# Sukikui/PTI-LDM-VAE

Hardware: AMD Instinct MI355X
Metric: vae_train_images_per_sec_256x256 (higher is better)
Workload: dtype fp16 forward operands + activations / bf16 backward operands + gradients, fp32 accumulate; 1 GPU; config/vae_dente_no_adv.json 256x256x1 batch 32/GPU: fwd + L1 + 1e-3*KL + bwd + all-reduce + Adam (perceptual term omitted: --perceptual times it; adversarial branch inactive before epoch 6, --adv times it); global_batch=32, parallelism=dp1

## Files before the change

### include/pti_vae.h

```cpp
#ifndef PTI_VAE_H
#define PTI_VAE_H

#include <stdint.h>

#ifdef __cplusplus
extern "C" {
#endif

typedef void* pti_stream_t;

#define PTI_ABI_VERSION 5

#define PTI_OK 0
#define PTI_EINVAL (-1)
#define PTI_EUNSUPPORTED (-2)
#define PTI_ELAUNCH (-3)

#define PTI_CONV_S1 0
#define PTI_CONV_S2PAD 1
#define PTI_CONV_UP2 2
#define PTI_CONV_ZINS 3

#define PTI_PRO_NONE 0
#define PTI_PRO_GN 1
#define PTI_PRO_GN_SILU 2

typedef struct pti_conv_desc {
  int32_t n, h, w, cin;
  int32_t ho, wo, cout;
  int32_t ksize;
  int32_t mode;
  int32_t prologue;
  int32_t groups;
  int32_t add_residual;
  int32_t accum_stats;
  int32_t out_groups;
  float eps;
  int32_t in_f32;
  int32_t out_f32;
  int64_t in_stride[4];
  int64_t out_stride[4];
  int32_t in_f16, res_f16, out_f16;
  int32_t pool2x2_out;
  int32_t w_f16;
  int32_t relu_out;
} pti_conv_desc;

int pti_abi_version(void);
const char* pti_last_error_string(void);
const char* pti_last_kernel_name(void);

int64_t pti_conv_packed_bytes(int cout, int cin, int ksize, int mode);
int pti_conv_pack_weights(const float* const* w_oihw, int nsrc, void* packed, int cout, int cin,
                          int ksize, int mode, int transpose_flip, int w_f16, pti_stream_t s);

int pti_conv_pack_entry_bytes(void);
int pti_conv_pack_table_fill(void* host_entry, const float* w_oihw_dev, void* packed_dev, int cout,
                             int cin, int ksize, int mode, int transpose_flip, int w_f16, int64_t* nblocks);
int pti_conv_pack_weights_batched(const void* table_dev, const int* blk_first_dev, int n,
                                  int total_blocks, pti_stream_t s);

int pti_gn_stats(const void* x_nhwc_16bit, int64_t* stats, int n, int hw, int c, int groups,
                 int x_f16, pti_stream_t s);

int pti_conv2d_mfma(const void* x, const void* w_packed, const float* bias, const int64_t* in_stats,
                    const float* gamma, const float* beta, const void* residual, void* y,
                    int64_t* out_stats, const pti_conv_desc* d, pti_stream_t s);

int pti_conv2d_mfma_saveact(const void* x, const void* w_packed, const float* bias, const int64_t* in_stats,
                            const float* gamma, const float* beta, const void* residual, void* y,
                            int64_t* out_stats, void* act_out, const pti_conv_desc* d, pti_stream_t s);

int pti_conv2d_direct(const void* x, const float* w_tck, const float* bias, const int64_t* in_stats,
                      const float* gamma, const float* beta, void* y, const pti_conv_desc* d,
                      pti_stream_t s);

#define PTI_DIRECT_REPACK_MAX 8
typedef struct {
  const float* w; const float* b;
  float* w_tck; float* w_tck_t; float* wpad; float* bpad;
  int cout, cin, pad_cin, reserved;
} pti_direct_repack_entry;
typedef struct {
  pti_direct_repack_entry e[PTI_DIRECT_REPACK_MAX];
  int n;
} pti_direct_repack_table;
int pti_direct_repack(const pti_direct_repack_table* t, pti_stream_t s);

int pti_wgrad_direct(const void* wide, const void* narrow, float* dw, float* dbias_wide,
                     float* dbias_narrow, const int64_t* in_stats, const float* gamma,
                     const float* beta, int n, int h, int w, int cw, int cn, int ksize, int sgn,
                     int prologue, int groups, float eps, int narrow_f32, int wide_f16,
                     const int64_t* narrow_stride, int64_t dw_stride_tap, int64_t dw_stride_cw,
                     int64_t dw_stride_k, void* workspace, int64_t workspace_bytes, pti_stream_t s);

int64_t pti_conv_wgrad_workspace_bytes(int cout, int cin, int ksize, int splits);
int pti_conv_wgrad_mfma(const void* x, const void* dy, const int64_t* in_stats, const float* gamma,
                        const float* beta, float* dw, float* dbias, void* workspace,
                        int64_t workspace_bytes, int accumulate, const pti_conv_desc* d,
                        pti_stream_t s);
int pti_conv_wgrad_mfma_partials(const void* x, const void* dy, const int64_t* in_stats,
                                 const float* gamma, const float* beta, void* workspace,
                                 int64_t workspace_bytes, const pti_conv_desc* d, int* splits_out,
                                 pti_stream_t s);
int pti_conv_wgrad_reduce(const void* workspace, int splits, float* dw, float* dbias,
                          int accumulate, const pti_conv_desc* d, pti_stream_t s);

#define PTI_WGRAD_BATCH_MAX 16
typedef struct pti_wgrad_job {
  const void* x;
  const void* dy;
  float* dw;
  float* dbias;
  int32_t n, h, w, cin, cout;
  int32_t accumulate;
} pti_wgrad_job;
int pti_conv_wgrad_mfma_batched(const pti_wgrad_job* jobs, int njobs, void* workspace, int64_t workspace_bytes,
                                pti_stream_t s);
int pti_conv_wgrad_batched_mode(int n, int h, int w, int cin, int cout);

int pti_gn_bwd_blocks(int n, int hw, int c);
int pti_gn_bwd(const void* x, const void* da, const void* dres, void* dx, const int64_t* stats,
               const float* gamma, const float* beta, float* sums, float* partials, float* dgamma,
               float* dbeta, int n, int hw, int c, int groups, float eps, int silu, int x_f16,
               pti_stream_t s);
int pti_conv_gnbwd_tiles(const pti_conv_desc* d);
int pti_conv_gnbwd_chain_supported(int cin, int cout, int ksize);
int pti_conv2d_mfma_gnbwd_chain(const void* g_in, const void* x_in, int x_in_f16, const int64_t* in_stats,
                                const float* in_gamma, const float* in_sums, void* dx_in_out, const void* w_packed,
                                const void* gx, const int64_t* gstats, const float* ggamma, const float* gbeta,
                                void* dy_out, float* gsums, const pti_conv_desc* d, int silu, pti_stream_t s);
int pti_gn_affine_grads(const float* sums, float* dgamma, float* dbeta, int n, int c, pti_stream_t s);
int pti_gn_sums_finalize_affine(const float* partials, float* sums, int n, int tiles, int row_len, const float* affine_sums,
                                float* dgamma, float* dbeta, int affine_c, pti_stream_t s);
int pti_conv2d_mfma_gnbwd(const void* dy_in, const void* w_packed, const void* gx, const int64_t* gstats,
                          const float* ggamma, const float* gbeta, void* dy_out, float* gpartials,
                          const pti_conv_desc* d, int silu, pti_stream_t s);
int pti_gn_sums_finalize(const float* partials, float* sums, int n, int tiles, int row_len,
                         pti_stream_t s);
int pti_gn_bwd_apply(const void* x, const void* dy, const void* dres, void* dx, const int64_t* stats,
                     const float* gamma, const float* beta, const float* sums, float* dgamma,
                     float* dbeta, int n, int hw, int c, int groups, float eps, int x_f16,
                     pti_stream_t s);
int pti_pool2x2_sum(const void* x, void* y, int n, int h, int w, int c, pti_stream_t s);

int pti_attention_fwd(const void* qkv, void* o, float* lse2, int b, int l, int c, pti_stream_t s);
int pti_attention_bwd(const void* qkv, const void* o, const void* dout, const float* lse2,
                      float* delta, void* dqkv, int b, int l, int c, pti_stream_t s);

int pti_latent_head_fwd(const float* h, const float* eps, const float* wm, const float* bm,
                        const float* wl, const float* bl, const float* wp, const float* bp,
                        float* mu, float* sigma, float* logvar, float* zq, int b, int hw, int l,
                        pti_stream_t s);
int pti_post_quant(const float* z_nchw, const float* wp, const float* bp, float* zq_nhwc, int b,
                   int hw, int l, pti_stream_t s);
#define PTI_POST_QUANT_BWD_MAX_BLOCKS 256
#define PTI_POST_QUANT_BWD_WS_FLOATS(l) (PTI_POST_QUANT_BWD_MAX_BLOCKS * ((l) * (l) + (l)))
int pti_post_quant_bwd(const float* dzq_nhwc, const float* z_nchw, const float* wp, float* dz_nchw,
                       float* gwp, float* gbp, float* workspace, int b, int hw, int l,
                       pti_stream_t s);
#define PTI_LATENT_BWD_MAX_BLOCKS 512
#define PTI_LATENT_BWD_WS_FLOATS(l) (PTI_LATENT_BWD_MAX_BLOCKS * 3 * ((l) * (l) + (l)))
int pti_latent_head_bwd(const float* h, const float* eps, const float* wm, const float* bm,
                        const float* wl, const float* bl, const float* wp, const float* bp,
                        const float* dzq, const float* dmu, const float* dsigma, float* dh,
                        float* gwm, float* gbm, float* gwl, float* gbl, float* gwp, float* gbp,
                        float* workspace, int b, int hw, int l, pti_stream_t s);

#define PTI_VAE_LOSS_MAX_BLOCKS 1024
#define PTI_VAE_LOSS_WS_FLOATS (2 * PTI_VAE_LOSS_MAX_BLOCKS)
int pti_vae_loss(const float* recon, const float* images, int64_t npix, const float* mu,
                 const float* third, int64_t nlat, int batch, float* out2, float* d_recon,
                 float* d_mu, float* d_third, float* workspace, int l2, int third_mode,
                 float kl_weight, pti_stream_t s);
// ... 184 lines not shown
```

### pti_ldm_vae_amd/_lib.py

```python
from __future__ import annotations

import ctypes as C
import os

_HERE = os.path.dirname(os.path.abspath(__file__))
LIB_PATH = os.environ.get("PTI_VAE_LIB") or os.path.join(_HERE, "libpti_vae_hip.so")

def env_overrides() -> dict:
    return {k: v for k, v in sorted(os.environ.items()) if k.startswith("PTI_")}


def refuse_wrong_result_env(who: str) -> None:
    bad = [k for k in os.environ if k.startswith("PTI_") and ("DIAG" in k or k == "PTI_ALLOW_WRONG_RESULTS")]
    if bad:
        raise SystemExit(f"{who}: refusing to run with wrong-result diagnostic variable(s) set: {sorted(bad)} "
                         "(timing diagnostics live in tools/diag_skip.py)")


ABI_VERSION = 5
PTI_CONV_S1, PTI_CONV_S2PAD, PTI_CONV_UP2, PTI_CONV_ZINS = 0, 1, 2, 3
PTI_PRO_NONE, PTI_PRO_GN, PTI_PRO_GN_SILU = 0, 1, 2


class ConvDesc(C.Structure):

    _fields_ = [
        ("n", C.c_int32), ("h", C.c_int32), ("w", C.c_int32), ("cin", C.c_int32),
        ("ho", C.c_int32), ("wo", C.c_int32), ("cout", C.c_int32),
        ("ksize", C.c_int32), ("mode", C.c_int32), ("prologue", C.c_int32), ("groups", C.c_int32),
        ("add_residual", C.c_int32), ("accum_stats", C.c_int32), ("out_groups", C.c_int32),
        ("eps", C.c_float), ("in_f32", C.c_int32), ("out_f32", C.c_int32),
        ("in_stride", C.c_int64 * 4), ("out_stride", C.c_int64 * 4),
        ("in_f16", C.c_int32), ("res_f16", C.c_int32), ("out_f16", C.c_int32), ("pool2x2_out", C.c_int32),
        ("w_f16", C.c_int32), ("relu_out", C.c_int32),
    ]


class WgradJob(C.Structure):

    _fields_ = [("x", C.c_void_p), ("dy", C.c_void_p), ("dw", C.c_void_p), ("dbias", C.c_void_p),
                ("n", C.c_int32), ("h", C.c_int32), ("w", C.c_int32), ("cin", C.c_int32), ("cout", C.c_int32),
                ("accumulate", C.c_int32)]


WGRAD_BATCH_MAX = 16
DIRECT_REPACK_MAX = 8
MASK_COMPARE_COLUMNS = ("n_gt", "n_pred", "components_gt", "components_pred", "kept_gt", "kept_pred", "filled_pred",
                        "intersection", "union", "gt_x", "gt_y", "gt_w", "gt_h", "pred_x", "pred_y", "pred_w", "pred_h",
                        "gt_width_upper", "gt_width_middle", "gt_width_lower",
                        "pred_width_upper", "pred_width_middle", "pred_width_lower", "status")
MASK_MOMENTS_COLUMNS = ("m00", "m10", "m01", "m20", "m11", "m02", "A", "B", "C", "status")
ALIGN_BOTTOM_COLUMNS = ("centre_gt", "centre_pred", "count_gt", "count_pred", "shift", "status")
GRAD_GUARD_COLUMNS = ("applied_steps", "skipped_steps", "sumsq", "norm", "coef", "skip", "bias1", "bias2_sqrt",
                      "ema_decay", "grad_mul")
GRAD_GUARD_HOST_COLUMNS = 8
GRAD_GUARD_PARTIALS_CAP = 1024


class DirectRepackEntry(C.Structure):

    _fields_ = [("w", C.c_void_p), ("b", C.c_void_p), ("w_tck", C.c_void_p), ("w_tck_t", C.c_void_p), ("wpad", C.c_void_p),
                ("bpad", C.c_void_p), ("cout", C.c_int32), ("cin", C.c_int32), ("pad_cin", C.c_int32), ("reserved", C.c_int32)]


class DirectRepackTable(C.Structure):

    _fields_ = [("e", DirectRepackEntry * DIRECT_REPACK_MAX), ("n", C.c_int32)]


_P = C.c_void_p
_I = C.c_int
_I64 = C.c_int64
_F = C.c_float
_D = C.c_double
_U32 = C.c_uint32

SIGNATURES = {
    "pti_abi_version": (_I, []),
    "pti_last_error_string": (C.c_char_p, []),
    "pti_last_kernel_name": (C.c_char_p, []),
    "pti_conv_packed_bytes": (_I64, [_I, _I, _I, _I]),
    "pti_conv_pack_weights": (_I, [C.POINTER(_P), _I, _P, _I, _I, _I, _I, _I, _I, _P]),
    "pti_conv_pack_entry_bytes": (_I, []),
    "pti_conv_pack_table_fill": (_I, [_P, _P, _P, _I, _I, _I, _I, _I, _I, C.POINTER(_I64)]),
    "pti_conv_pack_weights_batched": (_I, [_P, _P, _I, _I, _P]),
    "pti_gn_stats": (_I, [_P, _P, _I, _I, _I, _I, _I, _P]),
    "pti_conv2d_mfma": (_I, [_P, _P, _P, _P, _P, _P, _P, _P, _P, C.POINTER(ConvDesc), _P]),
    "pti_conv2d_mfma_saveact": (_I, [_P, _P, _P, _P, _P, _P, _P, _P, _P, _P, C.POINTER(ConvDesc), _P]),
    "pti_conv2d_direct": (_I, [_P, _P, _P, _P, _P, _P, _P, C.POINTER(ConvDesc), _P]),
    "pti_wgrad_direct": (_I, [_P, _P, _P, _P, _P, _P, _P, _P, _I, _I, _I, _I, _I, _I, _I, _I, _I, _F, _I, _I,
                              C.POINTER(_I64), _I64, _I64, _I64, _P, _I64, _P]),
    "pti_conv_wgrad_workspace_bytes": (_I64, [_I, _I, _I, _I]),
    "pti_conv_wgrad_mfma": (_I, [_P, _P, _P, _P, _P, _P, _P, _P, _I64, _I, C.POINTER(ConvDesc), _P]),
    "pti_conv_wgrad_mfma_partials": (_I, [_P, _P, _P, _P, _P, _P, _I64, C.POINTER(ConvDesc), C.POINTER(_I), _P]),
    "pti_conv_wgrad_mfma_batched": (_I, [C.POINTER(WgradJob), _I, _P, _I64, _P]),
    "pti_conv_wgrad_batched_mode": (_I, [_I, _I, _I, _I, _I]),
    "pti_direct_repack": (_I, [C.POINTER(DirectRepackTable), _P]),
    "pti_conv_wgrad_reduce": (_I, [_P, _I, _P, _P, _I, C.POINTER(ConvDesc), _P]),
    "pti_gn_bwd_blocks": (_I, [_I, _I, _I]),
    "pti_gn_bwd": (_I, [_P, _P, _P, _P, _P, _P, _P, _P, _P, _P, _P, _I, _I, _I, _I, _F, _I, _I, _P]),
    "pti_conv_gnbwd_tiles": (_I, [C.POINTER(ConvDesc)]),
    "pti_gn_sums_finalize": (_I, [_P, _P, _I, _I, _I, _P]),
    "pti_conv2d_mfma_gnbwd": (_I, [_P, _P, _P, _P, _P, _P, _P, _P, C.POINTER(ConvDesc), _I, _P]),
    "pti_conv_gnbwd_chain_supported": (_I, [_I, _I, _I]),
    "pti_conv2d_mfma_gnbwd_chain": (_I, [_P, _P, _I, _P, _P, _P, _P, _P, _P, _P, _P, _P, _P, _P, C.POINTER(ConvDesc), _I, _P]),
    "pti_gn_affine_grads": (_I, [_P, _P, _P, _I, _I, _P]),
    "pti_gn_sums_finalize_affine": (_I, [_P, _P, _I, _I, _I, _P, _P, _P, _I, _P]),
    "pti_gn_bwd_apply": (_I, [_P, _P, _P, _P, _P, _P, _P, _P, _P, _P, _I, _I, _I, _I, _F, _I, _P]),
    "pti_pool2x2_sum": (_I, [_P, _P, _I, _I, _I, _I, _P]),
    "pti_attention_fwd": (_I, [_P, _P, _P, _I, _I, _I, _P]),
    "pti_attention_bwd": (_I, [_P, _P, _P, _P, _P, _P, _I, _I, _I, _P]),
    "pti_latent_head_fwd": (_I, [_P] * 12 + [_I, _I, _I, _P]),
    "pti_post_quant": (_I, [_P, _P, _P, _P, _I, _I, _I, _P]),
    "pti_post_quant_bwd": (_I, [_P, _P, _P, _P, _P, _P, _P, _I, _I, _I, _P]),
    "pti_latent_head_bwd": (_I, [_P] * 19 + [_I, _I, _I, _P]),
    "pti_vae_loss": (_I, [_P, _P, _I64, _P, _P, _I64, _I, _P, _P, _P, _P, _P, _I, _I, _F, _P]),
    "pti_ar_vae_loss": (_I, [_P, _I, _I, _I, _P, _P, _P, _I, _P, _F, _P, _P, _P, _P]),
    "pti_pd_im2col_image": (_I, [_P, _P, _I, _I, _I, _P]),
    "pti_pd_im2col": (_I, [_P, _P, _P, _I, _I, _I, _I, _I, _I, _F, _P]),
    "pti_pd_in_stats": (_I, [_P, _P, _I, _I, _I, _F, _P]),
    "pti_pd_col2im_blocks": (_I, [_I, _I, _I]),
    "pti_pd_col2im": (_I, [_P, _P, _P, _P, _P, _I, _I, _I, _I, _I, _F, _P]),
    "pti_pd_col2im_image": (_I, [_P, _P, _I, _I, _I, _F, _I, _P]),
    "pti_pd_in_bwd_apply": (_I, [_P, _P, _P, _P, _P, _I, _I, _I, _P]),
    "pti_pd_lsgan_blocks": (_I, [_I]),
    "pti_pd_lsgan": (_I, [_P, _I, _I, _I, _F, _F, _F, _P, _P, _P]),
    "pti_pd_final_fwd": (_I, [_P, _P, _P, _P, _P, _I, _I, _I, _I, _F, _P]),
    "pti_pd_final_dgrad": (_I, [_P, _P, _P, _P, _P, _P, _I, _I, _I, _I, _F, _P]),
    "pti_pd_final_wgrad_blocks": (_I, [_I, _I, _I]),
    "pti_pd_final_wgrad": (_I, [_P, _P, _P, _P, _I, _I, _I, _I, _F, _P]),
    "pti_lpips_tap_blocks": (_I, [_I, _I]),
    "pti_lpips_tap_fwd": (_I, [_P, _P, _P, _P, _P, _I, _I, _I, _P]),
    "pti_lpips_tap_bwd": (_I, [_P, _P, _P, _P, _P, _P, _I, _I, _I, _P]),
    "pti_relu_f16": (_I, [_P, _I64, _P]),
    "pti_relu_bwd": (_I, [_P, _P, _I64, _P]),
    "pti_relu_bwd_add": (_I, [_P, _P, _P, _I64, _P]),
    "pti_maxpool3s2_out": (_I, [_I]),
    "pti_maxpool3s2_fwd": (_I, [_P, _P, _I, _I, _I, _I, _P]),
    "pti_maxpool3s2_bwd": (_I, [_P, _P, _P, _P, _I, _I, _I, _I, _I, _P]),
    "pti_squeeze_conv1_fwd": (_I, [_P, _P, _P, _I, _I, _I, _P]),
    "pti_squeeze_conv1_bwd": (_I, [_P, _P, _P, _P, _I, _I, _I, _P]),
    "pti_nchw_f32_to_nhwc_f16": (_I, [_P, _P, _I, _I, _I, _P]),
    "pti_pad_nchw_to_nhwc32": (_I, [_P, _P, _P, _I, _I, _I, _I, _I, _P]),
    "pti_slice_nhwc32_to_nchw": (_I, [_P, _P, _I, _I, _I, _I, _P]),
    "pti_nhwc_bf16_add_to_nchw_f32": (_I, [_P, _P, _I, _I, _I, _P]),
    "pti_lpips_tap_nhwc_blocks": (_I, [_I, _I]),
    "pti_lpips_tap_nhwc_fwd": (_I, [_P, _P, _P, _P, _P, _I, _I, _I, _P]),
    "pti_lpips_tap_nhwc_bwd": (_I, [_P, _P, _P, _P, _P, _P, _I, _I, _I, _P]),
    "pti_adam_step": (_I, [_P, _P, _P, _P, _I64, _F, _F, _F, _F, _I, _F, _P]),
    "pti_grad_guard_partials": (_I, [_I64]),
    "pti_grad_guard": (_I, [_P, _I64, _D, _D, _I, _F, _F, _D, _P, _P, _P]),
    "pti_adam_step_guarded": (_I, [_P, _P, _P, _P, _P, _I64, _F, _F, _F, _F, _P, _P]),
    "pti_preprocess_batch": (_I, [_P, _P, _P, _I, _I, _I, _P, _P, _P]),
    "pti_cast_nchw_f32_to_nhwc_bf16": (_I, [_P, _P, _I, _I, _I, _P]),
    "pti_cast_nhwc_bf16_to_nchw_f32": (_I, [_P, _P, _I, _I, _I, _P]),
    "pti_image_metrics_ws_floats": (_I64, [_I, _I, _I, _I]),
    "pti_image_metrics": (_I, [_P, _P, _I, _I, _I, _I, _I, _F, _F, _F, _F, _F, _P, _P, _P, _P]),
    "pti_latent_pairwise_ws_floats": (_I64, [_I, _I, _I]),
    "pti_latent_pairwise": (_I, [_P, _I64, _I, _P, _I64, _I, _I, _P, _I, _P, _I64, _P, _P]),
    "pti_latent_group_stats_ws_floats": (_I64, [_I, _I, _I, _I]),
    "pti_latent_group_stats": (_I, [_P, _I64, _I, _P, _P, _I64, _I, _P, _I, _I, _P, _P, _P]),
    "pti_mask_geometry": (_I, [_P, _P, _P, _I, _I, _I, _P, _I, _P, _I, _P, _P, _P, _P]),
    "pti_mlp_head_ws_floats": (_I64, [_I, _I, C.POINTER(C.c_int32), _I]),
    "pti_mlp_head_fwd": (_I, [_P, _I64, _I, _I, _P, C.POINTER(C.c_int32), _I, _I, _P, _P, _P, _I, _P, _P, _P, _P]),
    "pti_regression_metrics": (_I, [_P, _P, _P, _I, _I, _I, _P, _P]),
    "pti_elastic_field": (_I, [_P, _P, _F, _I, _I, _I, _P, _P]),
    "pti_augment_warp": (_I, [_P, _P, _P, _I, _I, _I, _I, _P, _P]),
    "pti_tsne_affinities_ws_floats": (_I64, [_I]),
    "pti_tsne_affinities": (_I, [_P, _I64, _I, _F, _P, _I64, _P, _P, _P]),
    "pti_tsne_step_ws_floats": (_I64, [_I, _I]),
    "pti_tsne_step": (_I, [_P, _I64, _I, _I, _P, _P, _P, _P, _P, _F, _F, _F, _P, _I, _P, _P]),
    "pti_umap_knn": (_I, [_P, _I64, _I, _I, _P, _P, _P]),
    "pti_umap_graph_capacity": (_I64, [_I, _I]),
# ... 65 lines not shown
```

### pti_ldm_vae_amd/csrc/conv_mfma.hip

```cpp
#include "conv_common.h"

namespace {
using namespace pti_conv;

constexpr int TH = 8, TW = 16;

__host__ __device__ constexpr int pick_cout_tile(int cout) { return cout % 128 == 0 ? 128 : (cout % 64 == 0 ? 64 : 32); }
__host__ __device__ constexpr int pick_ck(int cin, int stride2) {
  int ck = cin % 128 == 0 ? 128 : (cin % 64 == 0 ? 64 : 32);
  return (stride2 && ck > 64) ? 64 : ck;
}
__host__ __device__ constexpr int pick_wblk(int kbc, int nt) {
  int best = 1;
  for (int w = 1; w <= kbc; ++w)
    if (kbc % w == 0 && w * nt <= 16) best = w;
  return best;
}

template <int KS, int S, int CK, int COUT_TILE>
struct Cfg {
  static constexpr int HH = (TH - 1) * S + KS, HW = (TW - 1) * S + KS;
  static constexpr int NP = HH * HW;
  static constexpr int NC = CK / 8;
  static constexpr int PIXB = CK * 2;
// ... 112 lines not shown
      const int vy = vy0 + hy, vx = vx0 + hx;
      bool v = (p < C::NP) && vy >= 0 && vy < VH && vx >= 0 && vx < VW;
      int iy = vy, ix = vx;
      if (twox) {
        if (a.mode == PTI_CONV_ZINS) v = v && !((vy | vx) & 1);
        iy = vy >> 1;
        ix = vx >> 1;
      }
      ok[it] = v;
      raw[it] = u32x4{0u, 0u, 0u, 0u};
      if (v) raw[it] = *(const u32x4*)(a.x + ((size_t)(n * a.H + iy) * a.W + ix) * a.Cin + chunk * CK + lc * 8);
    }
#pragma unroll
    for (int it = 0; it < C::HITERS; ++it) {
      const int p = lp0 + it * PSTEP;
      if (p < C::NP) {
        const int hy = p / C::HW, hx = p - hy * C::HW;
        u32x4 r = raw[it];
        if (a.prologue != PTI_PRO_NONE && ok[it]) {
          float f[8];
          unpack8f(r, f, a.in_f16);
#pragma unroll
          for (int j = 0; j < 8; ++j) {
            float v = f[j] * sc[j] + sh[j];
            if (a.prologue == PTI_PRO_GN_SILU) v = silu_f(v);
            f[j] = v;
          }
          r = OPH ? pack8f(f, true) : pack8(f);
        } else if (a.in_f16 && !OPH) {
          float f[8];
          unpack8f(r, f, true);
          r = pack8(f);
        }
        const int key = (hx >> C::KEY_SHIFT) & (C::NC - 1);
        *(u32x4*)(halo + p * C::PIXB + ((lc ^ key) << 4)) = r;
      }
    }
    __syncthreads();

#pragma unroll
    for (int s = 0; s < C::NSTEP; ++s) {
      const int g = chunk * C::NSTEP + s;
      const bool more = (g + 1 < total_steps);
      if (more) wload(g + 1);
      const unsigned char* wcur = wbuf + (g & 1) * C::STEPB;
#pragma unroll
      for (int kbl = 0; kbl < C::WBLK; ++kbl) {
        constexpr int dummy = 0;
        (void)dummy;
        const int kb = s * C::WBLK + kbl;
        const int tap = kb / C::KPC, kc = kb % C::KPC;
        const int kh = tap / KS, kw = tap % KS;
        bf16x8 bfrag[C::PXF], afrag[C::CF];
#pragma unroll
        for (int i = 0; i < C::PXF; ++i)
          bfrag[i] = *(const bf16x8*)(halo + pbase[i][kw] + kh * C::HW * C::PIXB + ((kc * 32) ^ tkey[kw]));
#pragma unroll
        for (int c = 0; c < C::CF; ++c)
          afrag[c] = *(const bf16x8*)(wcur + ((kbl * C::NT + wn * C::CF + c) * 64 + lane) * 16);
#pragma unroll
        for (int i = 0; i < C::PXF; ++i)
#pragma unroll
          for (int c = 0; c < C::CF; ++c)
            acc[i][c] = mfma32<OPH>(afrag[c], bfrag[i], acc[i][c]);
      }
      if (more) wstore((g + 1) & 1);
      __syncthreads();
    }
  }

  const int j = lane & 31;
  stat_t* sstat = reinterpret_cast<stat_t*>(smem);
  const bool do_stats = a.out_stats != nullptr;
  const int ocpg = do_stats ? a.Cout / a.out_groups : 1;
  if (do_stats) {
    if (tid < 2 * a.out_groups) sstat[tid] = 0;
    __syncthreads();
  }
#pragma unroll
  for (int i = 0; i < C::PXF; ++i) {
    const int ty = 2 * (wm * C::PXF + i) + (j >> 4), tx = j & 15;
    const int oy = oy0 + ty, ox = ox0 + tx;
    const bool inb = (oy < a.Ho) && (ox < a.Wo);
    const size_t pix = ((size_t)(n * a.Ho + oy) * a.Wo + ox) * a.Cout;
#pragma unroll
    for (int c = 0; c < C::CF; ++c) {
#pragma unroll
      for (int q = 0; q < 4; ++q) {
        const int co = ct * COUT_TILE + (wn * C::CF + c) * 32 + 8 * q + 4 * hsel;
        float v0 = acc[i][c][4 * q + 0], v1 = acc[i][c][4 * q + 1], v2 = acc[i][c][4 * q + 2],
              v3 = acc[i][c][4 * q + 3];
        if (a.bias) {
          const f32x4 b = *(const f32x4*)(a.bias + co);
          v0 += b[0]; v1 += b[1]; v2 += b[2]; v3 += b[3];
        }
        u32x2 packed = u32x2{0u, 0u};
        if (inb) {
          if (a.res) {
            const u32x2 rr = *(const u32x2*)(a.res + pix + co);
            float e0, e1, e2, e3;
            unpack2f(rr[0], a.res_f16, e0, e1);
            unpack2f(rr[1], a.res_f16, e2, e3);
            v0 += e0; v1 += e1; v2 += e2; v3 += e3;
          }
          packed = pack4f(v0, v1, v2, v3, a.out_f16);
          *(u32x2*)(a.y + pix + co) = packed;
        }
        if (do_stats) {
          float r0, r1, r2, r3;
          unpack2f(packed[0], a.out_f16, r0, r1);
          unpack2f(packed[1], a.out_f16, r2, r3);
          if (!inb) r0 = r1 = r2 = r3 = 0.f;
          if (ocpg >= 4) {
            float s1 = (r0 + r1) + (r2 + r3), s2 = (r0 * r0 + r1 * r1) + (r2 * r2 + r3 * r3);
#pragma unroll
            for (int o = 16; o > 0; o >>= 1) {
              s1 += __shfl_xor(s1, o, 64);
              s2 += __shfl_xor(s2, o, 64);
            }
            if (j == 0) {
              const int g = co / ocpg;
              stat_add(&sstat[2 * g], s1);
              stat_add(&sstat[2 * g + 1], s2);
            }
          } else {
            float a1 = r0 + r1, a2 = r0 * r0 + r1 * r1, b1 = r2 + r3, b2 = r2 * r2 + r3 * r3;
#pragma unroll
            for (int o = 16; o > 0; o >>= 1) {
              a1 += __shfl_xor(a1, o, 64);
              a2 += __shfl_xor(a2, o, 64);
              b1 += __shfl_xor(b1, o, 64);
              b2 += __shfl_xor(b2, o, 64);
            }
            if (j == 0) {
              const int g = co / 2;
              stat_add(&sstat[2 * g], a1);
              stat_add(&sstat[2 * g + 1], a2);
              stat_add(&sstat[2 * g + 2], b1);
              stat_add(&sstat[2 * g + 3], b2);
            }
          }
        }
      }
    }
  }
  if (do_stats) {
    __syncthreads();
    const int g0 = (ct * COUT_TILE) / ocpg, ng = COUT_TILE / ocpg;
    if (tid < 2 * ng)
      atomicAdd((unsigned long long*)&a.out_stats[(n * a.out_groups + g0) * 2 + tid], (unsigned long long)sstat[2 * g0 + tid]);
  }
}

template <int KS, int CK, int CT, int PXF, bool SAVE, int FM, int PRO>
__global__ __launch_bounds__(256, (PXF == 2 ? 4 : 2)) void conv_mfma2_kernel(ConvArgs a) {
  using C = Cfg2<KS, CK, CT, PXF>;
  const int prologue = PRO >= 0 ? PRO : a.prologue;
  const bool gn_on = FM == 3 ? true : (FM == 0 ? a.gn_mode != 0 : false);
  const bool in_f16 = FM == 0 ? (bool)a.in_f16 : (FM == 1);
  const bool res_f16 = FM == 0 ? (bool)a.res_f16 : (FM == 1 || FM == 3);
  const bool out_f16 = FM == 0 ? (bool)a.out_f16 : (FM == 1);
  constexpr bool OPH = (FM == 1);
  if (out_f16) fp16_saturate_on();
  __shared__ __attribute__((aligned(16))) unsigned char smem[C::LDS_BYTES];
  unsigned char* halo = smem;
  const int tid = threadIdx.x, lane = tid & 63, wave = tid >> 6;
  const int hsel = lane >> 5;
  int t = blockIdx.x;
  const int tile_x = t % a.tiles_x;
  t /= a.tiles_x;
  const int tile_y = t % a.tiles_y;
  const int n = t / a.tiles_y;
  const int oy0 = tile_y * C::TH2, ox0 = tile_x * C::TW2;
  const int ct = blockIdx.y;
  const int nchunks = a.Cin / CK;
  const int wm = wave / C::WN, wn = wave % C::WN;

  const int pad_lo = (a.mode == PTI_CONV_ZINS) ? 2 : (KS - 1) / 2;
  const int vy0 = oy0 - pad_lo, vx0 = ox0 - pad_lo;
  const bool twox = (a.mode == PTI_CONV_UP2) || (a.mode == PTI_CONV_ZINS);
  const int VH = twox ? 2 * a.H : a.H, VW = twox ? 2 * a.W : a.W;

  int pbase[KS], tkey[KS];
  {
    const int j = lane & 31, tx = j & 15, row0 = 2 * PXF * wm + (j >> 4);
#pragma unroll
    for (int kw = 0; kw < KS; ++kw) {
      const int hx = tx + kw;
      tkey[kw] = (hsel ^ ((hx >> C::KEY_SHIFT) & (C::NC - 1))) << 4;
      pbase[kw] = (row0 * C::HW + hx) * C::PIXB;
    }
  }
  f32x16 acc[PXF];
#pragma unroll
  for (int i = 0; i < PXF; ++i)
#pragma unroll
    for (int r = 0; r < 16; ++r) acc[i][r] = 0.f;

  const int lc = tid % C::NC, lp0 = tid / C::NC;
  constexpr int PSTEP = 256 / C::NC;
  const int cpg = a.Cin / (a.groups > 0 ? a.groups : 1);
  reinterpret_cast<float*>(smem + C::STAT_OFF)[tid] = 0.f;
  float* sfl = reinterpret_cast<float*>(smem + C::STAT_OFF + 1024);
  if (prologue == PTI_PRO_GN || prologue == PTI_PRO_GN_SILU) {
    if (tid < 2 * a.groups) sfl[tid] = stat_f(a.in_stats, n * a.groups * 2 + tid);
  } else if (gn_on) {
    if (tid < 2 * a.g_groups) sfl[tid] = stat_f(a.g_stats, n * a.g_groups * 2 + tid);
  }
  float gq = 0.f, bq = 0.f;
  if (gn_on) {
    if (tid < CT) {
      gq = a.g_gamma[ct * CT + tid];
      bq = a.g_beta[ct * CT + tid];
    }
  } else if (a.bias) {
    if (tid < CT) reinterpret_cast<float*>(smem + C::BIAS_OFF)[tid] = a.bias[ct * CT + tid];
  }
  if (a.res) {
#pragma unroll
    for (int it = 0; it < C::EITERS; ++it) {
      const int slot = it * 256 + tid;
      const int p = slot / C::ENC, c = slot % C::ENC;
      const int oy = oy0 + p / C::TW2, ox = ox0 + p % C::TW2;
      if (oy < a.Ho && ox < a.Wo) {
        const bf16* src = a.res + ((size_t)(n * a.Ho + oy) * a.Wo + ox) * a.Cout + ct * CT + ((c ^ ((p >> 2) & (C::ENC - 1))) << 3);
        __builtin_amdgcn_global_load_lds((const __attribute__((address_space(1))) void*)src,
                                         (__attribute__((address_space(3))) void*)(smem + C::RT_OFF + (it * 256 + wave * 64) * 16),
                                         16, 0, 0);
      }
    }
  }

  const int epc = tid % C::ENC, epp0 = tid / C::ENC;
  constexpr int EPSTEP = 256 / C::ENC;

  for (int chunk = 0; chunk < nchunks; ++chunk) {
    const unsigned char* wlane =
        a.w + ((size_t)(ct * nchunks + chunk) * C::KBC * C::NT + wn) * 1024 + lane * 16;
    bf16x8 wa[C::R], wb[C::R];
    auto wload = [&](bf16x8 (&dst)[C::R], int g) {
#pragma unroll
      for (int u = 0; u < C::R; ++u) {
        int kb = g * C::R + u;
        kb = kb < C::KBC ? kb : C::KBC - 1;
        dst[u] = *(const bf16x8*)(wlane + (size_t)kb * C::NT * 1024);
      }
    };
    constexpr bool WLATE = (SAVE && PXF == 2) || PRO == PRO_GNB;
    if constexpr (!WLATE) wload(wa, 0);

    u32x4 raw[C::HITERS];
    u32x4 raw2[PRO == PRO_GNB ? C::HITERS : 1];
    bool ok[C::HITERS];
    {
      const __amdgpu_buffer_rsrc_t xrs = __builtin_amdgcn_make_buffer_rsrc(
          const_cast<bf16*>(a.x), 0, (unsigned)a.N * (unsigned)a.H * (unsigned)a.W * (unsigned)a.Cin * 2u, 0x00020000);
      const __amdgpu_buffer_rsrc_t x2rs = __builtin_amdgcn_make_buffer_rsrc(
          const_cast<bf16*>(PRO == PRO_GNB ? a.x2 : a.x), 0, (unsigned)a.N * (unsigned)a.H * (unsigned)a.W * (unsigned)a.Cin * 2u, 0x00020000);
      const unsigned base = ((unsigned)n * a.H * a.W * a.Cin + chunk * CK + lc * 8) * 2u;
      const unsigned rowb = (unsigned)a.W * a.Cin * 2u, pixb = (unsigned)a.Cin * 2u;
#pragma unroll
      for (int it = 0; it < C::HITERS; ++it) {
        const int p = lp0 + it * PSTEP;
        const int hy = p / C::HW, hx = p - hy * C::HW;
        const int vy = vy0 + hy, vx = vx0 + hx;
        bool v = (p < C::NP) && (unsigned)vy < (unsigned)VH && (unsigned)vx < (unsigned)VW;
        int iy = vy, ix = vx;
        if (twox) {
          if (a.mode == PTI_CONV_ZINS) v = v && !((vy | vx) & 1);
          iy = vy >> 1;
          ix = vx >> 1;
        }
        ok[it] = v;
        const unsigned off = v ? base + (unsigned)iy * rowb + (unsigned)ix * pixb : 0x80000000u;
        raw[it] = __builtin_bit_cast(u32x4, __builtin_amdgcn_raw_buffer_load_b128(xrs, off, 0, 0));
        if constexpr (PRO == PRO_GNB) raw2[it] = __builtin_bit_cast(u32x4, __builtin_amdgcn_raw_buffer_load_b128(x2rs, off, 0, 0));
      }
    }
    if (chunk == 0) __syncthreads();
    float sc[8], sh[8];
    [[maybe_unused]] float gnb_b = 0.f, gnb_d = 0.f;
    if constexpr (PRO == PRO_GNB) {
      const int ch0 = chunk * CK + lc * 8, g = ch0 / cpg;
      const float mean = stat_f(a.in_stats, (n * a.groups + g) * 2) * a.inv_cnt;
      const float rstd = rsqrtf(fmaxf(stat_f(a.in_stats, (n * a.groups + g) * 2 + 1) * a.inv_cnt - mean * mean, 0.f) + a.eps);
      float t1 = 0.f, t2 = 0.f;
      for (int cc = g * cpg; cc < (g + 1) * cpg; ++cc) {
        const f32x2 sv = *(const f32x2*)(a.p_sums + ((size_t)n * a.Cin + cc) * 2);
        const float gm = a.gamma[cc];
        t1 += gm * sv[0];
        t2 += gm * sv[1];
      }
      const float c1 = t1 * a.inv_cnt, c2 = t2 * a.inv_cnt;
#pragma unroll
      for (int j = 0; j < 8; ++j) sc[j] = rstd * a.gamma[ch0 + j];
      gnb_b = -rstd * rstd * c2;
      gnb_d = -rstd * c1 - gnb_b * mean;
    } else if (prologue != PTI_PRO_NONE) {
      float mu_[8], rs_[8];
      gn_params<8>(sfl, a.gamma, a.beta, chunk * CK + lc * 8, cpg, a.inv_cnt, a.eps, sc, sh, mu_, rs_);
    }
    if (chunk > 0) __syncthreads();
#pragma unroll
    for (int it = 0; it < C::HITERS; ++it) {
      const int p = lp0 + it * PSTEP;
      if (p < C::NP) {
        const int hy = p / C::HW, hx = p - hy * C::HW;
        u32x4 r = raw[it];
        if constexpr (PRO == PRO_GNB) {
          if (ok[it]) {
            float f[8], h[8];
            unpack8(r, f);
            unpack8f(raw2[it], h, a.x2_f16 != 0);
#pragma unroll
            for (int j = 0; j < 8; ++j) f[j] = fmaf(sc[j], f[j], fmaf(gnb_b, h[j], gnb_d));
            r = pack8(f);
          }
        } else if (prologue != PTI_PRO_NONE && ok[it]) {
          float f[8];
          unpack8f(r, f, in_f16);
          if (PXF == 4 && prologue == PTI_PRO_GN_SILU) {
#pragma unroll
            for (int j = 0; j < 8; j += 2) {
              const f32x2 o = gn_silu2(f32x2{f[j], f[j + 1]}, f32x2{sc[j], sc[j + 1]}, f32x2{sh[j], sh[j + 1]});
              f[j] = o[0];
              f[j + 1] = o[1];
            }
          } else {
#pragma unroll
            for (int j = 0; j < 8; ++j) {
              float v = f[j] * sc[j] + sh[j];
              if (prologue == PTI_PRO_GN_SILU) v = silu_f(v);
              f[j] = v;
            }
          }
          r = OPH ? pack8f(f, true) : pack8(f);
        } else if (in_f16 && !OPH) {
          float f[8];
          unpack8f(r, f, true);
          r = pack8(f);
        }
        const int key = (hx >> C::KEY_SHIFT) & (C::NC - 1);
        *(u32x4*)(halo + p * C::PIXB + ((lc ^ key) << 4)) = r;
      }
    }
    __syncthreads();

    if constexpr (SAVE) {
      if (ct == 0) {
        constexpr int PL = (KS - 1) / 2;
        constexpr int SITERS = C::TH2 * C::TW2 * C::NC / 256;
        const __amdgpu_buffer_rsrc_t srs = __builtin_amdgcn_make_buffer_rsrc(
            a.act_out, 0, (unsigned)a.N * (unsigned)a.H * (unsigned)a.W * (unsigned)a.Cin * 2u, 0x00020000);
#pragma unroll 1
        for (int it = 0; it < SITERS; ++it) {
          const int idx = tid + it * 256;
          const int c8 = idx % C::NC, pi = idx / C::NC;
          const int hy = pi / C::TW2 + PL, hx = pi % C::TW2 + PL;
          const int vy = vy0 + hy, vx = vx0 + hx;
          if (vy < a.H && vx < a.W) {
            const int key = (hx >> C::KEY_SHIFT) & (C::NC - 1);
            u32x4 piece = *(const u32x4*)(halo + (hy * C::HW + hx) * C::PIXB + ((c8 ^ key) << 4));
            if constexpr (OPH) {
              float f[8];
              unpack8f(piece, f, true);
              piece = pack8(f);
            }
            __builtin_amdgcn_raw_buffer_store_b128(__builtin_bit_cast(bu32x4, piece), srs,
                                                   ((unsigned)((n * a.H + vy) * a.W + vx) * a.Cin + chunk * CK + c8 * 8) * 2u, 0, 2 );
          }
        }
      }
    }

    if constexpr (WLATE) wload(wa, 0);
    const int txl = lane & 15;
    auto baddr = [&](int kb) -> const unsigned char* {
      kb = kb < C::KBC ? kb : C::KBC - 1;
      const int tap = kb / C::KPC, kc = kb - tap * C::KPC;
      const int kh = (KS == 3) ? tap / 3 : 0, kw = tap - kh * KS;
      const int hx = txl + kw;
      const int tk = (hsel ^ ((hx >> C::KEY_SHIFT) & (C::NC - 1))) << 4;
      return halo + pbase[0] + (kh * C::HW + kw) * C::PIXB + ((kc * 32) ^ tk);
    };
    bf16x8 b0[PXF], b1[PXF];
    auto bread = [&](bf16x8 (&dst)[PXF], int kb) {
      const unsigned char* bp = baddr(kb);
#pragma unroll
      for (int i = 0; i < PXF; ++i) dst[i] = *(const bf16x8*)(bp + 2 * i * C::HW * C::PIXB);
    };
    auto group = [&](const bf16x8 (&w)[C::R], int g) {
      const int kb0 = g * C::R;
#pragma unroll
      for (int u = 0; u < C::R; ++u) {
        if ((u & 1) == 0) {
          bread(b1, kb0 + u + 1);
#pragma unroll
          for (int i = 0; i < PXF; ++i) acc[i] = mfma32<OPH>(w[u], b0[i], acc[i]);
        } else {
          bread(b0, kb0 + u + 1);
#pragma unroll
          for (int i = 0; i < PXF; ++i) acc[i] = mfma32<OPH>(w[u], b1[i], acc[i]);
        }
      }
      if (C::R & 1) {
#pragma unroll
        for (int i = 0; i < PXF; ++i) b0[i] = b1[i];
      }
    };
    constexpr int NG = C::KBC / C::R;
    bread(b0, 0);
    if constexpr (NG == 1) {
      group(wa, 0);
    } else {
#pragma clang loop unroll(disable)
      for (int g = 0; g < NG; g += 2) {
        wload(wb, g + 1);
        group(wa, g);
        wload(wa, g + 2);
        group(wb, g + 1);
      }
    }
  }

  const int j = lane & 31;
  unsigned char* etile = smem;
  const bool do_stats = (FM == 2 || FM == 3) ? false : a.out_stats != nullptr;
  const int ocpg = do_stats ? a.Cout / a.out_groups : 1;
  __syncthreads();
  float* gtab = reinterpret_cast<float*>(smem + C::GT_OFF);
  if (gn_on) {
    if (tid < CT) {
      gtab[tid] = gq;
      gtab[CT + tid] = bq;
    }
    __syncthreads();
  }
  const unsigned char* rtile = smem + C::RT_OFF;
  const int col0 = wn * 32 + 4 * hsel;
  float st1[4] = {0.f, 0.f, 0.f, 0.f}, st2[4] = {0.f, 0.f, 0.f, 0.f};
  float su1[4] = {0.f, 0.f, 0.f, 0.f}, su2[4] = {0.f, 0.f, 0.f, 0.f};
  if (gn_on) {
    const int gcpg = a.Cout / a.g_groups;
    float* gsm = reinterpret_cast<float*>(smem + C::STAT_OFF);
    float L[32];
#pragma unroll
    for (int q = 0; q < 4; ++q) {
      const int col = col0 + 8 * q, ch0 = ct * CT + col;
      float scv[4], shv[4], muv[4], rsv[4], l1[4] = {0.f, 0.f, 0.f, 0.f}, l2[4] = {0.f, 0.f, 0.f, 0.f};
      gn_params<4>(sfl, gtab - ct * CT, gtab + CT - ct * CT, ch0, gcpg, a.g_inv_cnt, a.g_eps, scv, shv, muv, rsv);
      float nmr[4];
#pragma unroll
      for (int r = 0; r < 4; ++r) nmr[r] = -muv[r] * rsv[r];
#pragma unroll
      for (int i = 0; i < PXF; ++i) {
        const int p = (2 * PXF * wm + 2 * i + (j >> 4)) * 16 + (j & 15);
        const bool inb = (oy0 + (p >> 4) < a.Ho) && (ox0 + (p & 15) < a.Wo);
        unsigned char* ep = etile + p * C::EPITCH + col * 2;
        const u32x2 rr = *(const u32x2*)(rtile + p * (CT * 2) + ((((col >> 3) ^ (p >> 2)) & (C::ENC - 1)) << 4) + (col & 7) * 2);
        float xv[4];
        unpack2f(rr[0], res_f16, xv[0], xv[1]);
        unpack2f(rr[1], res_f16, xv[2], xv[3]);
        float dv[4];
#pragma unroll
        for (int r = 0; r < 4; ++r) {
          float v = acc[i][4 * q + r];
          if (a.gn_mode == 2) v *= dsilu_f(xv[r] * scv[r] + shv[r]);
          dv[r] = v;
        }
        const u32x2 packed = pack4(dv[0], dv[1], dv[2], dv[3]);
        *(u32x2*)ep = packed;
        if (inb) {
#pragma unroll
          for (int r = 0; r < 4; ++r) {
            l1[r] += dv[r];
            l2[r] = fmaf(dv[r], fmaf(xv[r], rsv[r], nmr[r]), l2[r]);
          }
        }
      }
#pragma unroll
      for (int r = 0; r < 4; ++r) {
        L[8 * q + 2 * r] = l1[r];
        L[8 * q + 2 * r + 1] = l2[r];
      }
    }
    fold32<32>(L, j);
    gsm[wm * 2 * CT + col0 * 2 + 16 * (j >> 3) + (j & 7)] = L[0];
  } else {
#pragma unroll
  for (int i = 0; i < PXF; ++i) {
    const int p = (2 * PXF * wm + 2 * i + (j >> 4)) * 16 + (j & 15);
    const bool inb = (oy0 + (p >> 4) < a.Ho) && (ox0 + (p & 15) < a.Wo);
#pragma unroll
    for (int q = 0; q < 4; ++q) {
      const int col = col0 + 8 * q;
      float v0 = acc[i][4 * q + 0], v1 = acc[i][4 * q + 1], v2 = acc[i][4 * q + 2], v3 = acc[i][4 * q + 3];
      if (a.bias) {
        const f32x4 b = *(const f32x4*)(smem + C::BIAS_OFF + col * 4);
        v0 += b[0]; v1 += b[1]; v2 += b[2]; v3 += b[3];
      }
      unsigned char* ep = etile + p * C::EPITCH + col * 2;
      if (a.res) {
        const u32x2 rr = *(const u32x2*)(rtile + p * (CT * 2) + ((((col >> 3) ^ (p >> 2)) & (C::ENC - 1)) << 4) + (col & 7) * 2);
        float e0, e1, e2, e3;
        unpack2f(rr[0], res_f16, e0, e1);
        unpack2f(rr[1], res_f16, e2, e3);
        v0 += e0; v1 += e1; v2 += e2; v3 += e3;
      }
      if constexpr (FM == 1 && PRO == PTI_PRO_NONE) {
        if (a.relu_out) { v0 = fmaxf(v0, 0.f); v1 = fmaxf(v1, 0.f); v2 = fmaxf(v2, 0.f); v3 = fmaxf(v3, 0.f); }
      }
      const u32x2 packed = pack4f(v0, v1, v2, v3, out_f16);
      *(u32x2*)ep = packed;
      if (do_stats && inb) {
        float r0, r1, r2, r3;
        unpack2f(packed[0], out_f16, r0, r1);
        unpack2f(packed[1], out_f16, r2, r3);
        if (ocpg >= 4) {
          st1[q] += (r0 + r1) + (r2 + r3);
          st2[q] += (r0 * r0 + r1 * r1) + (r2 * r2 + r3 * r3);
        } else {
          st1[q] += r0 + r1; st2[q] += r0 * r0 + r1 * r1;
          su1[q] += r2 + r3; su2[q] += r2 * r2 + r3 * r3;
        }
      }
    }
  }
  }
  if (do_stats) {
    stat_t* sstat = reinterpret_cast<stat_t*>(smem + C::STAT_OFF);
    if (ocpg >= 4) {
      float v[8];
#pragma unroll
      for (int q = 0; q < 4; ++q) { v[2 * q] = st1[q]; v[2 * q + 1] = st2[q]; }
      fold32<8>(v, j);
      if ((j & 3) == 0) {
        const int idx = j >> 2, q = idx >> 1;
        const int g = (ct * CT + col0 + 8 * q) / ocpg;
        stat_add(&sstat[2 * g + (idx & 1)], v[0]);
      }
    } else {
      float v[16];
#pragma unroll
      for (int q = 0; q < 4; ++q) { v[4 * q] = st1[q]; v[4 * q + 1] = st2[q]; v[4 * q + 2] = su1[q]; v[4 * q + 3] = su2[q]; }
      fold32<16>(v, j);
      if ((j & 1) == 0) {
        const int idx = j >> 1, q = idx >> 2;
        const int g = (ct * CT + col0 + 8 * q) / 2;
        stat_add(&sstat[2 * g + (idx & 3)], v[0]);
      }
    }
  }
  __syncthreads();
  const __amdgpu_buffer_rsrc_t yrs = __builtin_amdgcn_make_buffer_rsrc(
      a.y, 0, ((unsigned)a.N * (unsigned)a.Ho * (unsigned)a.Wo * (unsigned)a.Cout * 2u) >> (a.pool2 ? 2 : 0), 0x00020000);
  if ((FM == 0 || FM == 2) && a.pool2) {
    constexpr int PITERS = (C::EITERS + 3) / 4;
#pragma unroll
    for (int it = 0; it < PITERS; ++it) {
      const int idx = tid + it * 256;
      const int c8 = idx % C::ENC, pp = idx / C::ENC;
      const int py = pp / 8, px = pp % 8;
      const int oy = (oy0 >> 1) + py, ox = (ox0 >> 1) + px;
      if (pp < C::MPX / 4 && oy < (a.Ho >> 1) && ox < (a.Wo >> 1)) {
        const unsigned char* src = etile + ((2 * py) * 16 + 2 * px) * C::EPITCH + c8 * 16;
        float s_[8], f_[8];
        unpack8f(*(const u32x4*)src, s_, out_f16);
        unpack8f(*(const u32x4*)(src + C::EPITCH), f_, out_f16);
#pragma unroll
        for (int q = 0; q < 8; ++q) s_[q] += f_[q];
        unpack8f(*(const u32x4*)(src + 16 * C::EPITCH), f_, out_f16);
#pragma unroll
        for (int q = 0; q < 8; ++q) s_[q] += f_[q];
        unpack8f(*(const u32x4*)(src + 17 * C::EPITCH), f_, out_f16);
#pragma unroll
        for (int q = 0; q < 8; ++q) s_[q] += f_[q];
        __builtin_amdgcn_raw_buffer_store_b128(__builtin_bit_cast(bu32x4, pack8f(s_, out_f16)), yrs,
                                               ((unsigned)((n * (a.Ho >> 1) + oy) * (a.Wo >> 1) + ox) * a.Cout + ct * CT + c8 * 8) * 2u, 0, 2);
      }
    }
  } else
#pragma unroll
  for (int it = 0; it < C::EITERS; ++it) {
    const int p = epp0 + it * EPSTEP;
    const int oy = oy0 + (p >> 4), ox = ox0 + (p & 15);
    if (oy < a.Ho && ox < a.Wo)
      __builtin_amdgcn_raw_buffer_store_b128(__builtin_bit_cast(bu32x4, *(const u32x4*)(etile + p * C::EPITCH + epc * 16)), yrs,
                                             ((unsigned)((n * a.Ho + oy) * a.Wo + ox) * a.Cout + ct * CT + epc * 8) * 2u, 0, 2);
  }
  if (gn_on) {
    if (tid < 2 * CT) {
      const float* gsm = reinterpret_cast<const float*>(smem + C::STAT_OFF);
      float v = gsm[tid];
#pragma unroll
      for (int m = 1; m < C::WM; ++m) v += gsm[m * 2 * CT + tid];
      a.g_sums[(((size_t)n * a.g_T + tile_y * a.tiles_x + tile_x) * a.Cout + ct * CT) * 2 + tid] = v;
    }
  } else if (do_stats) {
    const stat_t* sstat = reinterpret_cast<const stat_t*>(smem + C::STAT_OFF);
    const int g0 = (ct * CT) / ocpg, ng = CT / ocpg;
    if (tid < 2 * ng)
      atomicAdd((unsigned long long*)&a.out_stats[(n * a.out_groups + g0) * 2 + tid], (unsigned long long)sstat[2 * g0 + tid]);
  }
}

template <int KS, int CK, int CT, int PXF>
int launch2_cfg(ConvArgs a, hipStream_t st) {
  using C = Cfg2<KS, CK, CT, PXF>;
  a.tiles_x = cdiv(a.Wo, C::TW2);
  a.tiles_y = cdiv(a.Ho, C::TH2);
  a.g_T = a.tiles_x * a.tiles_y;
  dim3 grid(a.N * a.tiles_x * a.tiles_y, a.Cout / CT);
  const bool res = a.res != nullptr;
  const int fm = (a.w_f16 && a.in_f16 && a.out_f16 && (a.res_f16 || !res)) ? 1
               : (!a.in_f16 && !a.out_f16 && (!a.res_f16 || !res)) ? 2
               : (!a.in_f16 && !a.out_f16 && a.res_f16) ? 3 : 0;
  const bool fwd_silu = fm == 1 && a.prologue == PTI_PRO_GN_SILU && !a.gn_mode && !a.pool2;
  const bool fwd_plain = fm == 1 && a.prologue == PTI_PRO_NONE && !a.gn_mode && !a.pool2;
  const bool dgrad = fm == 2 && a.prologue == PTI_PRO_NONE && !a.gn_mode && !a.out_stats;
  const bool dgrad_gn = fm == 3 && a.prologue == PTI_PRO_NONE && a.gn_mode && !a.out_stats && !a.pool2;
  if (a.x2) {
    if constexpr (KS == 3 && PXF == 4 && CT == 128) {
      if (!(fm == 3 && a.gn_mode && a.act_out && !a.out_stats && !a.pool2 && a.mode == PTI_CONV_S1 && !a.relu_out)) return 4;
      PTI_LAUNCH((conv_mfma2_kernel<KS, CK, CT, PXF, true, 3, PRO_GNB>), grid, dim3(256), 0, st, a);
      return 0;
    } else {
      return 4;
    }
  }
  if (a.relu_out && !(fwd_plain && !a.act_out)) return 3;
  constexpr int FPRO = PXF == 4 ? PTI_PRO_GN_SILU : -1;
  const bool fwd_gn_rt = fm == 1 && a.prologue == PTI_PRO_GN && !a.gn_mode && !a.pool2 && FPRO < 0;
  if constexpr (KS == 3) {
    if (a.act_out) {
      if (fwd_silu || fwd_gn_rt) PTI_LAUNCH((conv_mfma2_kernel<KS, CK, CT, PXF, true, 1, FPRO>), grid, dim3(256), 0, st, a);
      else if (a.w_f16) return 2;
      else PTI_LAUNCH((conv_mfma2_kernel<KS, CK, CT, PXF, true, 0, -1>), grid, dim3(256), 0, st, a);
      return 0;
    }
  } else if (a.act_out) {
    return 1;
  }
  if (fwd_silu) PTI_LAUNCH((conv_mfma2_kernel<KS, CK, CT, PXF, false, 1, FPRO>), grid, dim3(256), 0, st, a);
  else if (fwd_plain) PTI_LAUNCH((conv_mfma2_kernel<KS, CK, CT, PXF, false, 1, PTI_PRO_NONE>), grid, dim3(256), 0, st, a);
  else if (fm == 1 && !a.gn_mode && !a.pool2) PTI_LAUNCH((conv_mfma2_kernel<KS, CK, CT, PXF, false, 1, -1>), grid, dim3(256), 0, st, a);
  else if (a.w_f16) return 2;
  else if (dgrad) PTI_LAUNCH((conv_mfma2_kernel<KS, CK, CT, PXF, false, 2, PTI_PRO_NONE>), grid, dim3(256), 0, st, a);
  else if (dgrad_gn) PTI_LAUNCH((conv_mfma2_kernel<KS, CK, CT, PXF, false, 3, PTI_PRO_NONE>), grid, dim3(256), 0, st, a);
  else PTI_LAUNCH((conv_mfma2_kernel<KS, CK, CT, PXF, false, 0, -1>), grid, dim3(256), 0, st, a);
  return 0;
}
template <int KS>
int launch2(const ConvArgs& a, int ck, int ct, hipStream_t st) {
  if (ct == 128) {
    if (ck == 128) return launch2_cfg<KS, 128, 128, 4>(a, st);
    if (ck == 64) return launch2_cfg<KS, 64, 128, 4>(a, st);
    return launch2_cfg<KS, 32, 128, 4>(a, st);
  }
  if (ct == 64) {
    if (ck == 64) return launch2_cfg<KS, 64, 64, 2>(a, st);
    return launch2_cfg<KS, 32, 64, 2>(a, st);
  }
  return launch2_cfg<KS, 32, 32, 2>(a, st);
}

struct PackArgs {
  const float* src[4];
  int nsrc;
  bf16* dst;
  int cout_l, cin_l;
  int cout_o, cin_o;
  int ks, ck, cout_tile, flip;
  int f16;
  long long total;
};

__device__ __forceinline__ void pack_eight(const PackArgs& p, int e8) {
  const int NT = p.cout_tile / 32, KPC = p.ck / 16, KBC = p.ks * p.ks * KPC, nch = p.cin_l / p.ck;
  int r = e8;
  const int lane = r % 64; r /= 64;
  const int nt = r % NT; r /= NT;
  const int kb = r % KBC; r /= KBC;
  const int chunk = r % nch;
  const int ct = r / nch;
  const int co = ct * p.cout_tile + nt * 32 + (lane & 31);
  const int tap = kb / KPC, kc = kb % KPC;
  const int ci0 = chunk * p.ck + kc * 16 + 8 * (lane >> 5);
  const int kk = p.ks * p.ks;
  const float* src;
  size_t stride;
  if (!p.flip) {
    const int s_ = co / p.cout_o, cs = co % p.cout_o;
    src = p.src[s_] + ((size_t)cs * p.cin_o + ci0) * kk + tap;
    stride = kk;
  } else {
    src = p.src[0] + ((size_t)ci0 * p.cin_o + co) * kk + (kk - 1 - tap);
    stride = (size_t)p.cin_o * kk;
  }
  float f[8];
#pragma unroll
  for (int j = 0; j < 8; ++j) f[j] = src[j * stride];
  *(u32x4*)(p.dst + (size_t)e8 * 8) = p.f16 ? pack8f(f, true) : pack8(f);
}

__global__ void pack_weights_kernel(PackArgs p) {
  if (p.f16) fp16_saturate_on();
  const long long e8 = (long long)blockIdx.x * blockDim.x + threadIdx.x;
  if (e8 * 8 < p.total) pack_eight(p, (int)e8);
}

__global__ void pack_weights_batched_kernel(const PackArgs* __restrict__ table, const int* __restrict__ blk_first, int n) {
  int lo = 0, hi = n - 1;
  const int b = blockIdx.x;
  while (lo < hi) {
    const int mid = (lo + hi + 1) >> 1;
    if (blk_first[mid] <= b) lo = mid; else hi = mid - 1;
  }
  const PackArgs p = table[lo];
  if (p.f16) fp16_saturate_on();
  const int e8 = (b - blk_first[lo]) * 256 + threadIdx.x;
  if ((long long)e8 * 8 < p.total) pack_eight(p, e8);
}

template <int KS, int S, int CK, int COUT_TILE>
int launch_cfg(const ConvArgs& a, hipStream_t st) {
  dim3 grid(a.N * a.tiles_x * a.tiles_y, a.Cout / COUT_TILE);
  if (a.w_f16) PTI_LAUNCH((conv_mfma_kernel<KS, S, CK, COUT_TILE, true>), grid, dim3(256), 0, st, a);
  else PTI_LAUNCH((conv_mfma_kernel<KS, S, CK, COUT_TILE, false>), grid, dim3(256), 0, st, a);
  return 0;
}

template <int KS, int S, int CK>
int launch_ct(const ConvArgs& a, int cout_tile, hipStream_t st) {
  switch (cout_tile) {
    case 128: return launch_cfg<KS, S, CK, 128>(a, st);
    case 64: return launch_cfg<KS, S, CK, 64>(a, st);
    default: return launch_cfg<KS, S, CK, 32>(a, st);
  }
}

template <int KS, int S>
int launch_ck(const ConvArgs& a, int ck, int cout_tile, hipStream_t st) {
  static_assert(S == 2, "the v1 kernel is kept for the stride-2 gather only");
  switch (ck) {
    case 64: return launch_ct<KS, S, 64>(a, cout_tile, st);
    default: return launch_ct<KS, S, 32>(a, cout_tile, st);
  }
}

}

extern "C" int64_t pti_conv_packed_bytes(int cout, int cin, int ksize, int mode) {
  (void)mode;
  if (cout <= 0 || cin <= 0 || cout % 32 || cin % 32 || (ksize != 1 && ksize != 3)) return 0;
  return (int64_t)2 * cout * cin * ksize * ksize;
}

extern "C" int pti_conv_pack_weights(const float* const* w, int nsrc, void* packed, int cout, int cin,
                                     int ksize, int mode, int transpose_flip, int w_f16, pti_stream_t s) {
  if (!w || !packed || nsrc < 1 || nsrc > 4) PTI_FAIL(PTI_EINVAL, "pack_weights: bad pointer/nsrc");
  if (cout % 32 || cin % 32 || (ksize != 1 && ksize != 3))
    PTI_FAIL(PTI_EUNSUPPORTED, "pack_weights: cout=%d cin=%d k=%d need multiples of 32, k in {1,3}", cout, cin, ksize);
  if (transpose_flip && nsrc != 1) PTI_FAIL(PTI_EINVAL, "pack_weights: transpose_flip needs nsrc=1");
  PackArgs p;
  for (int i = 0; i < 4; ++i) p.src[i] = i < nsrc ? w[i] : nullptr;
  p.nsrc = nsrc;
  p.dst = (bf16*)packed;
  p.cout_o = cout;
  p.cin_o = cin;
  p.cout_l = transpose_flip ? cin : cout * nsrc;
  p.cin_l = transpose_flip ? cout : cin;
  p.ks = ksize;
  p.flip = transpose_flip;
  p.f16 = w_f16 ? 1 : 0;
  p.cout_tile = pick_cout_tile(p.cout_l);
  p.ck = (mode == PTI_CONV_S2PAD) ? pick_ck(p.cin_l, true) : pick_ck2(p.cin_l, p.cout_tile);
  p.total = (long long)p.cout_l * p.cin_l * ksize * ksize;
  const int blocks = (int)((p.total + 2047) / 2048);
  PTI_LAUNCH(pack_weights_kernel, dim3(blocks), dim3(256), 0, (hipStream_t)s, p);
  PTI_CHECK_LAUNCH("pack_weights");
  return PTI_OK;
}

static int fill_pack(PackArgs& p, const float* w, void* packed, int cout, int cin, int ksize, int mode, int flip, int f16) {
  if (cout % 32 || cin % 32 || (ksize != 1 && ksize != 3)) return -1;
  for (int i = 0; i < 4; ++i) p.src[i] = nullptr;
  p.src[0] = w;
  p.nsrc = 1;
  p.dst = (bf16*)packed;
  p.cout_o = cout; p.cin_o = cin;
  p.cout_l = flip ? cin : cout;
  p.cin_l = flip ? cout : cin;
  p.ks = ksize; p.flip = flip; p.f16 = f16 ? 1 : 0;
  p.cout_tile = pick_cout_tile(p.cout_l);
  p.ck = (mode == PTI_CONV_S2PAD) ? pick_ck(p.cin_l, true) : pick_ck2(p.cin_l, p.cout_tile);
  p.total = (long long)p.cout_l * p.cin_l * ksize * ksize;
  return 0;
}

extern "C" int pti_conv_pack_entry_bytes(void) { return (int)sizeof(PackArgs); }
extern "C" int pti_conv_pack_table_fill(void* host_entry, const float* w, void* packed, int cout, int cin, int ksize,
                                        int mode, int transpose_flip, int w_f16, int64_t* nblocks) {
  if (!host_entry || !w || !packed || !nblocks) PTI_FAIL(PTI_EINVAL, "pack_table_fill: null pointer");
  PackArgs p;
  if (fill_pack(p, w, packed, cout, cin, ksize, mode, transpose_flip, w_f16))
    PTI_FAIL(PTI_EUNSUPPORTED, "pack_table_fill: cout=%d cin=%d k=%d", cout, cin, ksize);
  *(PackArgs*)host_entry = p;
  *nblocks = (p.total + 2047) / 2048;
  return PTI_OK;
}
extern "C" int pti_conv_pack_weights_batched(const void* table_dev, const int* blk_first_dev, int n, int total_blocks,
                                             pti_stream_t s) {
  if (!table_dev || !blk_first_dev || n <= 0 || total_blocks <= 0) PTI_FAIL(PTI_EINVAL, "pack_weights_batched: bad args");
  PTI_LAUNCH(pack_weights_batched_kernel, dim3(total_blocks), dim3(256), 0, (hipStream_t)s,
                     (const PackArgs*)table_dev, blk_first_dev, n);
  PTI_CHECK_LAUNCH("pack_weights_batched");
  return PTI_OK;
}

struct GnBwdFuse {
  int mode; const int64_t* stats; const float* gamma; const float* beta; float* sums;
  const void* x2 = nullptr; int x2_f16 = 0; const int64_t* p_stats = nullptr; const float* p_gamma = nullptr; const float* p_sums = nullptr;
};

static int conv2d_mfma_impl(const void* x, const void* w_packed, const float* bias, const int64_t* in_stats,
                            const float* gamma, const float* beta, const void* residual, void* y,
                            int64_t* out_stats, const pti_conv_desc* d, const GnBwdFuse* gf, void* act_out,
                            pti_stream_t s) {
  if (!x || !w_packed || !y || !d) PTI_FAIL(PTI_EINVAL, "conv2d_mfma: null pointer");
  const bool chain = gf && gf->x2;
  if (act_out && !chain && (d->mode != PTI_CONV_S1 || d->prologue == PTI_PRO_NONE || d->ksize != 3))
    PTI_FAIL(PTI_EUNSUPPORTED, "conv2d_mfma: the activated-input side output needs a 3x3 PTI_CONV_S1 launch with a GroupNorm prologue");
  if (d->cin % 32 || d->cout % 32 || d->cin <= 0 || d->cout <= 0)
    PTI_FAIL(PTI_EUNSUPPORTED, "conv2d_mfma: cin=%d cout=%d must be positive multiples of 32", d->cin, d->cout);
  if (d->ksize != 1 && d->ksize != 3) PTI_FAIL(PTI_EUNSUPPORTED, "conv2d_mfma: ksize %d", d->ksize);
  if (d->ksize == 1 && d->mode != PTI_CONV_S1) PTI_FAIL(PTI_EUNSUPPORTED, "conv2d_mfma: 1x1 supports PTI_CONV_S1 only");
  if (d->n <= 0 || d->h <= 0 || d->w <= 0) PTI_FAIL(PTI_EINVAL, "conv2d_mfma: bad dims");
  int eho, ewo;
  switch (d->mode) {
    case PTI_CONV_S1: eho = d->h; ewo = d->w; break;
    case PTI_CONV_S2PAD: eho = (d->h + 1 - 3) / 2 + 1; ewo = (d->w + 1 - 3) / 2 + 1; break;
    case PTI_CONV_UP2: case PTI_CONV_ZINS: eho = 2 * d->h; ewo = 2 * d->w; break;
    default: PTI_FAIL(PTI_EUNSUPPORTED, "conv2d_mfma: mode %d", d->mode);
  }
  if (d->ho != eho || d->wo != ewo)
    PTI_FAIL(PTI_EINVAL, "conv2d_mfma: output %dx%d does not match mode %d on %dx%d (want %dx%d)", d->ho, d->wo,
             d->mode, d->h, d->w, eho, ewo);
  if (d->prologue != PTI_PRO_NONE) {
    if (!in_stats || !gamma || !beta || d->groups <= 0 || d->cin % d->groups)
      PTI_FAIL(PTI_EINVAL, "conv2d_mfma: prologue needs stats/gamma/beta and groups | cin");
    if (d->groups > 32) PTI_FAIL(PTI_EUNSUPPORTED, "conv2d_mfma: prologue supports at most 32 groups");
  }
  if (d->add_residual && !residual) PTI_FAIL(PTI_EINVAL, "conv2d_mfma: add_residual without residual");
  if (d->accum_stats) {
    if (!out_stats || d->out_groups <= 0 || d->cout % d->out_groups) PTI_FAIL(PTI_EINVAL, "conv2d_mfma: bad out stats");
    const int ocpg = d->cout / d->out_groups;
    if (ocpg != 2 && (ocpg % 4 != 0 || ocpg > 32)) PTI_FAIL(PTI_EUNSUPPORTED, "conv2d_mfma: channels/group %d for fused stats", ocpg);
    if (d->out_groups > 64) PTI_FAIL(PTI_EUNSUPPORTED, "conv2d_mfma: fused statistics support at most 64 groups");
  }
  ConvArgs a;
  a.x = (const bf16*)x; a.w = (const unsigned char*)w_packed; a.bias = bias; a.in_stats = (const stat_t*)in_stats;
  a.gamma = gamma; a.beta = beta; a.res = d->add_residual ? (const bf16*)residual : nullptr; a.y = (bf16*)y;
  a.out_stats = d->accum_stats ? (stat_t*)out_stats : nullptr;
  a.N = d->n; a.H = d->h; a.W = d->w; a.Cin = d->cin; a.Ho = d->ho; a.Wo = d->wo; a.Cout = d->cout;
  a.mode = d->mode; a.prologue = d->prologue; a.groups = d->groups; a.out_groups = d->out_groups;
  a.gn_mode = 0; a.g_groups = 0; a.g_inv_cnt = 0.f; a.g_eps = 0.f;
  a.g_stats = nullptr; a.g_gamma = a.g_beta = nullptr; a.g_sums = nullptr; a.g_T = 0;
  a.act_out = (bf16*)act_out;
  a.in_f16 = d->in_f16; a.res_f16 = d->res_f16; a.out_f16 = d->out_f16;
  a.pool2 = d->pool2x2_out;
  a.w_f16 = d->w_f16;
  a.relu_out = d->relu_out;
  if (a.relu_out && (gf || d->mode == PTI_CONV_S2PAD))
    PTI_FAIL(PTI_EUNSUPPORTED, "conv2d_mfma: relu_out is for plain fp16 forward launches (stride-1 gather, no prologue)");
  if (a.w_f16 && !(d->in_f16 && d->out_f16 && (d->res_f16 || !d->add_residual)) )
    PTI_FAIL(PTI_EUNSUPPORTED, "conv2d_mfma: fp16-packed weights need fp16 input, output and residual (the forward convs)");
  if (a.w_f16 && (gf || d->pool2x2_out))
    PTI_FAIL(PTI_EUNSUPPORTED, "conv2d_mfma: fp16-packed weights are for forward launches only");
  if (a.pool2 && (d->mode == PTI_CONV_S2PAD || d->accum_stats || gf || (d->ho & 1) || (d->wo & 1)))
    PTI_FAIL(PTI_EUNSUPPORTED, "conv2d_mfma: pool2x2_out needs a stride-1 gather, even output size, no fused statistics");
  a.eps = d->eps;
  a.inv_cnt = d->prologue != PTI_PRO_NONE ? 1.0f / ((float)(d->cin / d->groups) * (float)d->h * (float)d->w) : 0.f;
  if (gf) {
    if (d->groups > 32) PTI_FAIL(PTI_EUNSUPPORTED, "conv2d_mfma_gnbwd: at most 32 groups");
    a.gn_mode = gf->mode; a.g_groups = d->groups; a.g_eps = d->eps;
    a.g_inv_cnt = 1.0f / ((float)(d->cout / d->groups) * (float)d->ho * (float)d->wo);
    a.g_stats = (const stat_t*)gf->stats; a.g_gamma = gf->gamma; a.g_beta = gf->beta; a.g_sums = gf->sums;
  }
  a.x2 = nullptr; a.p_sums = nullptr; a.x2_f16 = 0;
  if (chain) {
    if (!gf->p_stats || !gf->p_gamma || !gf->p_sums || !act_out || d->mode != PTI_CONV_S1 || d->ksize != 3 ||
        d->cin % d->groups || d->cin / d->groups < 8)
      PTI_FAIL(PTI_EINVAL, "conv2d_mfma_gnbwd_chain: bad arguments (3x3 stride-1, >= 8 channels per group)");
    a.x2 = (const bf16*)gf->x2; a.x2_f16 = gf->x2_f16; a.p_sums = gf->p_sums;
    a.in_stats = (const stat_t*)gf->p_stats; a.gamma = gf->p_gamma; a.groups = d->groups;
    a.inv_cnt = 1.0f / ((float)(d->cin / d->groups) * (float)d->h * (float)d->w);
  }
  if ((long long)d->n * d->ho * d->wo * d->cout * 2 >= (1ll << 31))
    PTI_FAIL(PTI_EUNSUPPORTED, "conv2d_mfma: output tensor of %lld bytes (the stores use 32-bit offsets: < 2 GiB)",
             (long long)d->n * d->ho * d->wo * d->cout * 2);
  if (d->mode != PTI_CONV_S2PAD && (long long)d->n * d->h * d->w * d->cin * 2 >= (1ll << 31))
    PTI_FAIL(PTI_EUNSUPPORTED, "conv2d_mfma: input tensor of %lld bytes (the halo loads use 32-bit offsets: < 2 GiB)",
             (long long)d->n * d->h * d->w * d->cin * 2);
  a.tiles_x = cdiv(d->wo, TW); a.tiles_y = cdiv(d->ho, TH);
  const int cout_tile = pick_cout_tile(d->cout);
  int rc, ck;
  if (d->mode == PTI_CONV_S2PAD) {
    ck = pick_ck(d->cin, true);
    rc = launch_ck<3, 2>(a, ck, cout_tile, (hipStream_t)s);
  } else {
    ck = pick_ck2(d->cin, cout_tile);
    rc = (d->ksize == 3 && d->cin == 128 && d->cout == 128 && !a.x2) ? launch_conv_ws128(a, (hipStream_t)s) : 1;
    if (rc == 1)
      rc = d->ksize == 1 ? launch2<1>(a, ck, cout_tile, (hipStream_t)s) : launch2<3>(a, ck, cout_tile, (hipStream_t)s);
  }
  if (rc == 3) PTI_FAIL(PTI_EUNSUPPORTED, "conv2d_mfma: relu_out needs a plain fp16 forward launch (w_f16, fp16 in/out, no prologue, no side output)");
  if (rc == 2) PTI_FAIL(PTI_EUNSUPPORTED, "conv2d_mfma: no fp16-operand kernel for this launch (w_f16 with this prologue / epilogue)");
  if (rc == 4) PTI_FAIL(PTI_EUNSUPPORTED, "conv2d_mfma_gnbwd_chain: only 3x3 launches on 128-wide input and output tiles with an fp16 GroupNorm input");
  if (rc != 0) PTI_FAIL(PTI_EUNSUPPORTED, "conv2d_mfma: no kernel for ck=%d cout_tile=%d", ck, cout_tile);
  PTI_CHECK_LAUNCH("conv2d_mfma");
  return PTI_OK;
}

extern "C" int pti_conv2d_mfma(const void* x, const void* w_packed, const float* bias, const int64_t* in_stats,
                               const float* gamma, const float* beta, const void* residual, void* y,
                               int64_t* out_stats, const pti_conv_desc* d, pti_stream_t s) {
  return conv2d_mfma_impl(x, w_packed, bias, in_stats, gamma, beta, residual, y, out_stats, d, nullptr, nullptr, s);
}

extern "C" int pti_conv2d_mfma_saveact(const void* x, const void* w_packed, const float* bias, const int64_t* in_stats,
                                       const float* gamma, const float* beta, const void* residual, void* y,
                                       int64_t* out_stats, void* act_out, const pti_conv_desc* d, pti_stream_t s) {
  if (!act_out) PTI_FAIL(PTI_EINVAL, "conv2d_mfma_saveact: null act_out");
  return conv2d_mfma_impl(x, w_packed, bias, in_stats, gamma, beta, residual, y, out_stats, d, nullptr, act_out, s);
}

extern "C" int pti_conv_gnbwd_tiles(const pti_conv_desc* d) {
  if (!d || d->cout % 32 || d->ho <= 0 || d->wo <= 0) return 0;
  const int ct = pick_cout_tile(d->cout);
  const int th = ct == 128 ? 8 : (ct == 64 ? 8 : 16);
  return cdiv(d->ho, th) * cdiv(d->wo, 16);
}

extern "C" int pti_conv_gnbwd_chain_supported(int cin, int cout, int ksize) {
  return ksize == 3 && cin % 128 == 0 && cout % 128 == 0;
}

extern "C" int pti_conv2d_mfma_gnbwd_chain(const void* g_in, const void* x_in, int x_in_f16, const int64_t* in_stats,
                                           const float* in_gamma, const float* in_sums, void* dx_in_out, const void* w_packed,
                                           const void* gx, const int64_t* gstats, const float* ggamma, const float* gbeta,
                                           void* dy_out, float* gsums, const pti_conv_desc* d, int silu, pti_stream_t s) {
  if (!g_in || !x_in || !in_stats || !in_gamma || !in_sums || !dx_in_out || !gx || !gstats || !ggamma || !gbeta || !gsums || !d)
    PTI_FAIL(PTI_EINVAL, "conv2d_mfma_gnbwd_chain: null pointer");
  if (d->mode != PTI_CONV_S1 || d->prologue != PTI_PRO_NONE || d->add_residual || d->accum_stats)
    PTI_FAIL(PTI_EUNSUPPORTED, "conv2d_mfma_gnbwd_chain: plain stride-1 data-gradient launches only");
  if (d->groups <= 0 || d->cout % d->groups || d->cin % d->groups) PTI_FAIL(PTI_EINVAL, "conv2d_mfma_gnbwd_chain: groups must divide cin and cout");
  GnBwdFuse gf{silu ? 2 : 1, gstats, ggamma, gbeta, gsums};
  gf.x2 = x_in; gf.x2_f16 = x_in_f16; gf.p_stats = in_stats; gf.p_gamma = in_gamma; gf.p_sums = in_sums;
  pti_conv_desc dd = *d;
  dd.add_residual = 1;
  return conv2d_mfma_impl(g_in, w_packed, nullptr, nullptr, nullptr, nullptr, gx, dy_out, nullptr, &dd, &gf, dx_in_out, s);
}

extern "C" int pti_conv2d_mfma_gnbwd(const void* dy_in, const void* w_packed, const void* gx, const int64_t* gstats,
                                     const float* ggamma, const float* gbeta, void* dy_out, float* gsums,
                                     const pti_conv_desc* d, int silu, pti_stream_t s) {
  if (!gx || !gstats || !ggamma || !gbeta || !gsums || !d) PTI_FAIL(PTI_EINVAL, "conv2d_mfma_gnbwd: null pointer");
  if (d->mode == PTI_CONV_S2PAD || d->prologue != PTI_PRO_NONE || d->add_residual || d->accum_stats)
    PTI_FAIL(PTI_EUNSUPPORTED, "conv2d_mfma_gnbwd: plain stride-1 / zero-insert data-gradient launches only");
  if (d->groups <= 0 || d->cout % d->groups) PTI_FAIL(PTI_EINVAL, "conv2d_mfma_gnbwd: groups must divide cout");
  GnBwdFuse gf{silu ? 2 : 1, gstats, ggamma, gbeta, gsums};
  pti_conv_desc dd = *d;
  dd.add_residual = 1;
  return conv2d_mfma_impl(dy_in, w_packed, nullptr, nullptr, nullptr, nullptr, gx, dy_out, nullptr, &dd, &gf, nullptr, s);
}
```

### pti_ldm_vae_amd/engine.py

```python
from __future__ import annotations

import contextlib
import gc
import os
import warnings

import torch

from . import ops
from .models import autoencoderkl as M
from .ops import (BF16, F32, PTI_CONV_S1, PTI_CONV_S2PAD, PTI_CONV_UP2, PTI_CONV_ZINS, PTI_PRO_GN, PTI_PRO_GN_SILU,
                  PTI_PRO_NONE)


class _Act:

    __slots__ = ("t", "stats")

    def __init__(self, t, stats=None):
        self.t, self.stats = t, stats


def _empty(shape, like, dtype=BF16):
    return torch.empty(shape, dtype=dtype, device=like.device)


@contextlib.contextmanager
def gc_off_for_capture():
    gc.collect()
    enabled = gc.isenabled()
    gc.disable()
    try:
        yield
    finally:
        if enabled:
            gc.enable()


def capture_or_eager(what, *bodies):
    graphs, results = [], []
    try:
        with gc_off_for_capture():
            for body in bodies:
                g = torch.cuda.CUDAGraph()
                with torch.cuda.graph(g, pool=graphs[0].pool() if graphs else None, capture_error_mode="thread_local"):
                    results.append(body(*results))
                graphs.append(g)
    except Exception as ex:
        warnings.warn(f"HIP-graph capture of {what} failed ({ex!r}); continuing with eager launches")
        torch.cuda.synchronize()
        return None
    return graphs, results


class _MfmaConv:

    def __init__(self, net, wname, bname, ksize, mode, fused_names=None, fwd_f16=True):
        self.net, self.ksize, self.mode = net, ksize, mode
        self.fwd_f16, self.f16 = fwd_f16, False
        self.wname, self.bname, self.fused = wname, bname, fused_names
        if fused_names:
            w0 = net._param_by_name[fused_names[0][0]]
            self.cout, self.cin = 3 * w0.shape[0], w0.shape[1]
        else:
            w = net._param_by_name[wname]
            self.cout, self.cin = w.shape[0], w.shape[1]
        self.wp = self.wpt = None

    def _w(self):
        if self.fused:
            o, n, _ = self.net._slots[self.fused[0][0]]
            return self.net._arena[o:o + 3 * n].view(self.cout, self.cin, 1, 1)
        return self.net._param_by_name[self.wname].data.view(self.cout, self.cin, self.ksize, self.ksize)

    def bias(self):
        if self.fused:
            o, n, _ = self.net._slots[self.fused[0][1]]
            return self.net._arena[o:o + 3 * n]
        return self.net._param_by_name[self.bname].data

    def grads(self):
        if self.fused:
            o, n, _ = self.net._slots[self.fused[0][0]]
            ob, nb, _ = self.net._slots[self.fused[0][1]]
            g = self.net.grad_arena
            return g[o:o + 3 * n], g[ob:ob + 3 * nb]
        return self.net.grad_view(self.wname).view(-1), self.net.grad_view(self.bname)

    def fwd(self, x, *, pro=PTI_PRO_NONE, norm=None, residual=None, want_stats=False, eng=None, act_out=None,
            out_dtype=None):
        n, h, w, _ = x.t.shape
        ho, wo = ops.conv_out_hw(h, w, self.mode)
        y = _empty((n, ho, wo, self.cout), x.t, out_dtype or eng.act_dtype)
        st = eng.new_stats(n) if want_stats else None
        g, b = (norm.weight.data, norm.bias.data) if norm is not None else (None, None)
        ops.conv_mfma(x.t, self.wp, self.bias(), y, cout=self.cout, ksize=self.ksize, mode=self.mode, prologue=pro,
                      in_stats=x.stats if pro else None, gamma=g, beta=b, groups=eng.G, eps=eng.eps,
                      residual=residual, out_stats=st, out_groups=eng.G, act_out=act_out)
        return _Act(y, st)

    def dgrad(self, dy, *, residual=None):
        n, ho, wo, _ = dy.shape
        if self.mode == PTI_CONV_S2PAD:
            out = _empty((n, 2 * ho, 2 * wo, self.cin), dy)
            ops.conv_mfma(dy, self.wpt, None, out, cout=self.cin, ksize=3, mode=PTI_CONV_ZINS, residual=residual)
            return out
        if self.mode == PTI_CONV_UP2:
            pooled = _empty((n, ho // 2, wo // 2, self.cin), dy)
            ops.conv_mfma(dy, self.wpt, None, pooled, cout=self.cin, ksize=self.ksize, mode=PTI_CONV_S1, pool2=True)
            return pooled
        out = _empty((n, ho, wo, self.cin), dy)
        ops.conv_mfma(dy, self.wpt, None, out, cout=self.cin, ksize=self.ksize, mode=PTI_CONV_S1, residual=residual)
        return out

    def dgrad_gn(self, dy, x, norm, *, silu, dres, eng):
        g, sums = self.dgrad_gn_raw(dy, x, norm, silu=silu, eng=eng)
        return self._gn_apply(g, sums, x, norm, dres, eng)

    def _gn_apply(self, g, sums, x, norm, dres, eng):
        dx = _empty(x.t.shape, x.t)
        ops.gn_bwd_apply(x.t, g, dx, x.stats, norm.weight.data, norm.bias.data, sums,
                         norm.net.grad_view(norm.prefix + ".weight"), norm.net.grad_view(norm.prefix + ".bias"),
                         groups=eng.G, eps=eng.eps, dres=dres)
        return dx

    def dgrad_gn_raw(self, dy, x, norm, *, silu, eng):
        n, ho, wo, _ = dy.shape
        g = _empty((n, ho, wo, self.cin), dy)
        sums = eng.zeros(n * self.cin * 2)
        ops.conv_mfma_gnbwd(dy, self.wpt, x.t, x.stats, norm.weight.data, norm.bias.data, g, sums, cout=self.cin,
                            ksize=self.ksize, mode=PTI_CONV_S1, groups=eng.G, eps=eng.eps, silu=silu)
        return g, sums

    def dgrad_gn_chain(self, g_in, x_in, norm_in, sums_in, x, norm, *, silu, dres, eng):
        n, ho, wo, _ = g_in.shape
        dxin = _empty(g_in.shape, g_in)
        dyt = _empty((n, ho, wo, self.cin), g_in)
        sums = eng.zeros(n * self.cin * 2)
        ops.conv_mfma_gnbwd_chain(g_in, x_in.t, x_in.stats, norm_in.weight.data, sums_in, dxin, self.wpt, x.t, x.stats,
                                  norm.weight.data, norm.bias.data, dyt, sums, cout=self.cin, groups=eng.G, eps=eng.eps,
                                  silu=silu, in_dgamma=norm_in.net.grad_view(norm_in.prefix + ".weight"),
                                  in_dbeta=norm_in.net.grad_view(norm_in.prefix + ".bias"))
        return self._gn_apply(dyt, sums, x, norm, dres, eng), dxin

    def wgrad(self, x, dy, *, pro=PTI_PRO_NONE, norm=None, eng=None):
        dw, db = self.grads()
        if eng.batch_wgrad and ops.wgrad_batch_eligible(x.t, dy, self.ksize, self.mode, pro):
            eng.defer_wgrad(x.t, dy, dw, db)
            return
        g, b = (norm.weight.data, norm.bias.data) if norm is not None else (None, None)
        kw = dict(ksize=self.ksize, mode=self.mode, prologue=pro, in_stats=x.stats if pro else None, gamma=g, beta=b,
                  groups=eng.G, eps=eng.eps, accumulate=True)
        with eng.side_stream(x.t, dy, dw, db, *kw.values()) as workspace:
            ops.conv_wgrad_mfma(x.t, dy, dw, db, workspace=workspace, **kw)


class _Norm:
    def __init__(self, net, prefix):
        self.net, self.prefix = net, prefix
        self.weight = net._param_by_name[prefix + ".weight"]
        self.bias = net._param_by_name[prefix + ".bias"]

    def bwd(self, x, da, *, silu, dres, eng):
        n, h, w, c = x.t.shape
        dx = _empty(x.t.shape, x.t)
        sums = eng.zeros(n * c * 2)
        ops.gn_bwd(x.t, da, dx, x.stats, self.weight.data, self.bias.data, sums,
                   self.net.grad_view(self.prefix + ".weight"), self.net.grad_view(self.prefix + ".bias"),
                   groups=eng.G, eps=eng.eps, silu=silu, dres=dres)
        return dx


class _ResBlock:
    def __init__(self, net, p, blk):
        self.norm1, self.norm2 = _Norm(net, p + ".norm1"), _Norm(net, p + ".norm2")
        self.conv1 = _MfmaConv(net, p + ".conv1.conv.weight", p + ".conv1.conv.bias", 3, PTI_CONV_S1)
        self.conv2 = _MfmaConv(net, p + ".conv2.conv.weight", p + ".conv2.conv.bias", 3, PTI_CONV_S1)
        self.nin = None
        if blk.in_channels != blk.out_channels:
            self.nin = _MfmaConv(net, p + ".nin_shortcut.conv.weight", p + ".nin_shortcut.conv.bias", 1, PTI_CONV_S1)
        self.convs = [c for c in (self.conv1, self.conv2, self.nin) if c is not None]
        self.needs_in_stats = True
        self.prefix = p + "."

    def fwd(self, x, eng, want_stats, save):
        a1 = a2 = None
        if save is not None and eng.saves_activated_input(x.t):
            a1 = _empty(x.t.shape, x.t)
        h1 = self.conv1.fwd(x, pro=PTI_PRO_GN_SILU, norm=self.norm1, want_stats=True, eng=eng, act_out=a1)
        sc = x.t if self.nin is None else self.nin.fwd(x, eng=eng).t
        if save is not None and eng.saves_activated_input(h1.t):
            a2 = _empty(h1.t.shape, h1.t)
        out = self.conv2.fwd(h1, pro=PTI_PRO_GN_SILU, norm=self.norm2, residual=sc, want_stats=want_stats, eng=eng,
                             act_out=a2)
        if save is not None:
            save.append((x, h1, a1, a2))
        return out

    @staticmethod
    def _wgrad(conv, x, norm, a, dy, eng):
        if a is not None:
            conv.wgrad(_Act(a), dy, eng=eng)
        else:
            conv.wgrad(x, dy, pro=PTI_PRO_GN_SILU, norm=norm, eng=eng)

    def _shortcut_bwd(self, x, dout, eng):
        if self.nin is None:
            return dout
        dres = self.nin.dgrad(dout)
        self.nin.wgrad(x, dout, eng=eng)
        return dres

    def bwd(self, dout, saved, eng):
        x, h1, a1, a2 = saved
        self._wgrad(self.conv2, h1, self.norm2, a2, dout, eng)
        if eng.gnbwd_chain and ops.gnbwd_chain_supported(self.conv1.cout, self.conv1.cin, 3, x.t.dtype, eng.G):
            g2, sums2 = self.conv2.dgrad_gn_raw(dout, h1, self.norm2, silu=True, eng=eng)
            dres = self._shortcut_bwd(x, dout, eng)
            dx, dh1 = self.conv1.dgrad_gn_chain(g2, h1, self.norm2, sums2, x, self.norm1, silu=True, dres=dres, eng=eng)
            self._wgrad(self.conv1, x, self.norm1, a1, dh1, eng)
            return dx
        dh1 = self.conv2.dgrad_gn(dout, h1, self.norm2, silu=True, dres=None, eng=eng)
        self._wgrad(self.conv1, x, self.norm1, a1, dh1, eng)
        dres = self._shortcut_bwd(x, dout, eng)
        return self.conv1.dgrad_gn(dh1, x, self.norm1, silu=True, dres=dres, eng=eng)


class _Resample:

    def __init__(self, net, wprefix, mode, prefix):
        self.conv = _MfmaConv(net, wprefix + ".weight", wprefix + ".bias", 3, mode)
        self.convs = [self.conv]
        self.needs_in_stats = False
        self.prefix = prefix

    def fwd(self, x, eng, want_stats, save):
        out = self.conv.fwd(x, want_stats=want_stats, eng=eng)
        if save is not None:
            save.append(x)
        return out

    def bwd(self, dout, saved, eng):
        x = saved
        self.conv.wgrad(x, dout, eng=eng)
        return self.conv.dgrad(dout)


class _Attention:
    def __init__(self, net, p):
        self.norm = _Norm(net, p + ".norm")
        a = p + ".attn."
        self.qkv = _MfmaConv(net, None, None, 1, PTI_CONV_S1,
                             fused_names=[(a + "to_q.weight", a + "to_q.bias")], fwd_f16=False)
        self.proj = _MfmaConv(net, a + "out_proj.weight", a + "out_proj.bias", 1, PTI_CONV_S1, fwd_f16=False)
        self.convs = [self.qkv, self.proj]
        self.needs_in_stats = True
        self.prefix = p + "."

    def fwd(self, x, eng, want_stats, save):
        n, h, w, c = x.t.shape
        qkv = self.qkv.fwd(x, pro=PTI_PRO_GN, norm=self.norm, eng=eng, out_dtype=BF16).t
        o = _empty((n, h * w, c), x.t)
        lse = _empty((n, h * w), x.t, F32)
        ops.attention_fwd(qkv.view(n, h * w, 3 * c), o, lse)
        out = self.proj.fwd(_Act(o.view(n, h, w, c)), residual=x.t, want_stats=want_stats, eng=eng)
        if save is not None:
            save.append((x, qkv, o, lse))
        return out

    def bwd(self, dout, saved, eng):
        x, qkv, o, lse = saved
        n, h, w, c = x.t.shape
        do = self.proj.dgrad(dout)
        self.proj.wgrad(_Act(o.view(n, h, w, c)), dout, eng=eng)
        dqkv = _empty(qkv.shape, qkv)
        delta = _empty((n, h * w), qkv, F32)
        ops.attention_bwd(qkv.view(n, h * w, 3 * c), o, do.view(n, h * w, c), lse, delta, dqkv.view(n, h * w, 3 * c))
        self.qkv.wgrad(x, dqkv, pro=PTI_PRO_GN, norm=self.norm, eng=eng)
        return self.qkv.dgrad_gn(dqkv, x, self.norm, silu=False, dres=dout, eng=eng)


class _DirectConv:

    def __init__(self, net, prefix, norm_prefix=None):
        self.net, self.prefix = net, prefix
        self.w = net._param_by_name[prefix + ".weight"]
        self.b = net._param_by_name[prefix + ".bias"]
        self.cout, self.cin = self.w.shape[0], self.w.shape[1]
        self.norm = _Norm(net, norm_prefix) if norm_prefix else None
        self.few_cin = self.cin <= 16
        self.w_tck = self.w_tck_t = None
        self.convs = []
        self.needs_in_stats = self.norm is not None
        narrow, wide = min(self.cin, self.cout), max(self.cin, self.cout)
        self.mfma_narrow = 4 <= narrow <= 32 and wide % 32 == 0
        self.wpad = self.wp_mfma = None
        self.pack_f16 = False
        self.img_mfma = False
        self.wp_img = self.wpt_img = self.wpad_img = self.bpad_img = None
        self.dw_img = self.db_img = None

    def alloc(self):
        w = self.w.data
        if self.w_tck is not None:
            return
        self.w_tck = torch.empty(9, self.cin, self.cout, dtype=F32, device=w.device)
        self.w_tck_t = torch.empty(9, self.cout, self.cin, dtype=F32, device=w.device)
        if self.mfma_narrow:
            shape = (32, self.cin, 3, 3) if self.cout < self.cin else (self.cout, 32, 3, 3)
            self.wpad = torch.zeros(shape, dtype=F32, device=w.device)
            self.bpad = torch.zeros(32, dtype=F32, device=w.device)
        if self.img_mfma:
            shape = (self.cout, 32, 3, 3) if self.cin < self.cout else (32, self.cin, 3, 3)
            self.wpad_img = torch.zeros(shape, dtype=F32, device=w.device)
            self.bpad_img = torch.zeros(32, dtype=F32, device=w.device)
            self.dw_img = torch.zeros(shape, dtype=F32, device=w.device)
            self.db_img = torch.zeros(32, dtype=F32, device=w.device) if self.cout < self.cin else None

    def repack_entries(self):
        w, b = self.w.data, self.b.data
        out = [dict(w=w, b=b, w_tck=self.w_tck, w_tck_t=self.w_tck_t,
                    wpad=self.wpad, bpad=self.bpad if (self.mfma_narrow and self.cout < self.cin) else None)]
        if self.img_mfma:
            out.append(dict(w=w, b=b, wpad=self.wpad_img, bpad=self.bpad_img if self.cout < self.cin else None))
        return out

    def pack_entries(self):
        out = []
        if self.mfma_narrow:
            if self.cout < self.cin:
                out.append(("wp_mfma", (self.wpad, 3, PTI_CONV_S1, False, self.pack_f16)))
            else:
                out.append(("wp_mfma", (self.wpad, 3, PTI_CONV_S1, True, False)))
        if self.img_mfma:
            out.append(("wp_img", (self.wpad_img, 3, PTI_CONV_S1, False, self.pack_f16)))
            if self.cout < self.cin:
                out.append(("wpt_img", (self.wpad_img, 3, PTI_CONV_S1, True, False)))
        return out


class Engine:
    def __init__(self, net: "M.AutoencoderKL"):
        self.net = net
        self.G, self.eps = net.norm_num_groups, float(net.norm_eps)
        self.dev = net.param_arena.device
        self.workspace = ops.wgrad_workspace(self.dev)
        self.packed_version = -1
        self.pack_gen = 0
        self.grad_ready_cb = None
        self._range_cache = {}
        self._zpool, self._zoff, self._zpool_size = None, 0, 1 << 16
        self._packer = None
        self.save_act_min_hw = int(os.environ.get("PTI_SAVE_ACT_MIN_HW", "0"))
        self.act_dtype = {"fp16": torch.float16, "bf16": BF16}[os.environ.get("PTI_FWD_ACT_DTYPE", "fp16")]
        self.wgrad_stream = torch.cuda.Stream(device=self.dev) if os.environ.get("PTI_WGRAD_STREAM", "1") == "1" else None
        self.workspace_side = torch.empty_like(self.workspace) if self.wgrad_stream is not None else None
        self._wgrad_pending = False
        self._side_owned = set()
        self.wgrad_batch_max = max(1, min(ops.L.WGRAD_BATCH_MAX, int(os.environ.get("PTI_WGRAD_BATCH", "16"))))
        self.batch_wgrad = self.wgrad_batch_max > 1
        self._wgrad_jobs, self._ready_queue = [], []
        self.encode_graphs = os.environ.get("PTI_ENCODE_GRAPH", "1") == "1"
        self._enc_graphs, self._dec_graphs, self._enc_graph_version = {}, {}, None
        ops.L.lib()
        for c in net.channels:
            if c % 32:
                raise ValueError(f"HIP path needs channel counts that are multiples of 32, got {net.channels}")
            cpg = c // self.G
            if cpg not in (2, 4, 8, 16, 32) or (c & (c - 1)):
                raise ValueError(f"HIP GroupNorm path supports power-of-two channels with 2..32 channels per group; "
                                 f"got channels={c}, groups={self.G}")
        eb = net.encoder.blocks
        self.enc_in = _DirectConv(net, "encoder.blocks.0.conv")
        self.enc_layers = []
        last = len(eb) - 1
        for i in range(1, last - 1):
            self.enc_layers.append(self._make_layer(eb[i], f"encoder.blocks.{i}"))
        self.enc_out = _DirectConv(net, f"encoder.blocks.{last}.conv", norm_prefix=f"encoder.blocks.{last - 1}")
        db = net.decoder.blocks
        self.dec_in = _DirectConv(net, "decoder.blocks.0.conv")
        self.dec_layers = []
        last = len(db) - 1
        for i in range(1, last - 1):
            self.dec_layers.append(self._make_layer(db[i], f"decoder.blocks.{i}"))
        self.dec_out = _DirectConv(net, f"decoder.blocks.{last}.conv", norm_prefix=f"decoder.blocks.{last - 1}")
        self.mfma_convs = [c for l in self.enc_layers + self.dec_layers for c in l.convs]
        for c in self.mfma_convs:
            c.f16 = c.fwd_f16 and self.act_dtype == torch.float16
        self.direct_convs = [self.enc_in, self.enc_out, self.dec_in, self.dec_out]
        self.enc_out.pack_f16 = self.act_dtype == torch.float16
        img = os.environ.get("PTI_IMG_MFMA", "1") == "1"
        self.enc_in.img_mfma = img and 2 <= net.in_channels <= 8 and net.channels[0] % 32 == 0
        self.dec_out.img_mfma = img and 2 <= net.out_channels <= 8 and net.channels[0] % 32 == 0
        self.enc_in.pack_f16 = self.dec_out.pack_f16 = self.act_dtype == torch.float16
        self._wgrad_posts, self._wgrad_zero = [], ()
        self._flush_up = int(os.environ.get("PTI_WGRAD_FLUSH_UP", "1"))
        self.gnbwd_chain = os.environ.get("PTI_GNBWD_CHAIN", "0") == "1"
        self.Lc = net.latent_channels
        self._plist = list(net._param_by_name.values())

    def saves_activated_input(self, t) -> bool:
        return t.shape[1] * t.shape[2] >= self.save_act_min_hw

    def _make_layer(self, blk, prefix):
        if isinstance(blk, M.AEKLResBlock):
            return _ResBlock(self.net, prefix, blk)
        if isinstance(blk, M.AEKLDownsample):
            return _Resample(self.net, prefix + ".conv.conv", PTI_CONV_S2PAD, prefix + ".")
        if isinstance(blk, M.Upsample):
            return _Resample(self.net, prefix + ".postconv.conv", PTI_CONV_UP2, prefix + ".")
        if isinstance(blk, M.SpatialAttentionBlock):
            return _Attention(self.net, prefix)
        raise TypeError(f"unsupported block {type(blk)} at {prefix}")

    def new_stats(self, n):
        return self.zeros(n * self.G * 4).view(torch.int64).view(n, self.G, 2)

    def zeros(self, count):
        count = (count + 3) // 4 * 4
        pool = self._zpool
        if pool is None or self._zoff + count > pool.numel():
            pool = self._zpool = torch.zeros(max(count, self._zpool_size), dtype=F32, device=self.dev)
            self._zoff = 0
        out = pool[self._zoff:self._zoff + count]
        self._zoff += count
        return out

    def begin_pass(self, batch, backward=False):
        cmax = max(self.net.channels)
        self._zpool_size = (64 * batch * cmax * 2) if backward else (96 * batch * self.G * 2)
        self._zpool = None
        if backward and self.wgrad_stream is not None:
            self._side_owned = {t.untyped_storage().data_ptr()
                                for t in (self.net.param_arena, self.net.grad_arena, self.workspace_side)}

    def _pack_buffer_ids(self):
        ids = [t.data_ptr() for c in self.mfma_convs for t in (c.wp, c.wpt) if t is not None]
        for c in self.direct_convs:
            ids += [t.data_ptr() for t in (c.w_tck, c.w_tck_t, c.wp_mfma, c.wpad, c.wp_img, c.wpt_img, c.wpad_img) if t is not None]
        return tuple(ids)

    def _drop_stale_graphs(self):
        ids = self._pack_buffer_ids()
        if ids != self._enc_graph_version:
            self._enc_graphs.clear()
            self._dec_graphs.clear()
            self._enc_graph_version = ids

    def refresh_weights(self):
        v = sum(p._version for p in self._plist)
        if v == self.packed_version:
            return
        if self._packer is None:
            entries = []
            for c in self.mfma_convs:
                dmode = PTI_CONV_ZINS if c.mode == PTI_CONV_S2PAD else PTI_CONV_S1
                entries += [(c._w(), c.ksize, c.mode, False, c.f16), (c._w(), c.ksize, dmode, True, False)]
            rep, targets = [], []
            for c in self.direct_convs:
                c.alloc()
                rep += c.repack_entries()
                for attr, e in c.pack_entries():
                    targets.append((c, attr, len(entries)))
                    entries.append(e)
            self._direct_repack = ops.DirectRepack(rep)
            self._packer = ops.BatchedPacker(entries, self.dev)
            for i, c in enumerate(self.mfma_convs):
                c.wp, c.wpt = self._packer.outputs[2 * i], self._packer.outputs[2 * i + 1]
            for c, attr, i in targets:
                setattr(c, attr, self._packer.outputs[i])
        self._direct_repack.run()
        self._packer.run()
        self.packed_version = v
        self.pack_gen += 1

    def _qp(self, name):
        L = self.Lc
        w = self.net._param_by_name[name + ".conv.weight"].data.view(L, L)
        b = self.net._param_by_name[name + ".conv.bias"].data
        return w, b

    def _check_input(self, x, channels, what):
        if not x.is_cuda:
            raise RuntimeError(f"{what}: expected a cuda (HIP) tensor; the VAE hot path has no CPU fallback")
        if x.dim() != 4 or x.shape[1] != channels:
            raise ValueError(f"{what}: expected [B,{channels},H,W], got {tuple(x.shape)}")
        if x.dtype != F32:
            x = x.float()
        return x.contiguous()

    def _walk_fwd(self, layers, act, tail_needs_stats, save):
        for i, l in enumerate(layers):
            nxt_needs = layers[i + 1].needs_in_stats if i + 1 < len(layers) else tail_needs_stats
            act = l.fwd(act, self, nxt_needs, save)
        return act

    def _walk_bwd(self, layers, dout, saved):
        for l, s in zip(reversed(layers), reversed(saved)):
            dout = l.bwd(dout, s, self)
            self._ready(l.prefix)
        return dout

    @contextlib.contextmanager
    def side_stream(self, *operands):
        ws = self.wgrad_stream
        if ws is None:
            yield self.workspace
            return
        ev = torch.cuda.Event()
        ev.record(torch.cuda.current_stream())
        ws.wait_event(ev)
        self.record_side(*operands)
        with torch.cuda.stream(ws):
            yield self.workspace_side
        self._wgrad_pending = True

    def _wgrad_direct(self, wide, narrow, *args, **kw):
        with self.side_stream(wide, narrow, *args, *kw.values()) as workspace:
            ops.wgrad_direct(wide, narrow, *args, workspace=workspace, **kw)

    def record_side(self, *operands):
        ws = self.wgrad_stream
        owned = self._side_owned
        for t in operands:
            if isinstance(t, torch.Tensor) and t.untyped_storage().data_ptr() not in owned:
                t.record_stream(ws)

    def defer_wgrad(self, x, dy, dw, db, post=None, zero=()):
        if self._flush_up and self._wgrad_jobs:
            new, old = x.shape[1] * x.shape[2], self._wgrad_jobs[-1][0].shape[1] * self._wgrad_jobs[-1][0].shape[2]
            if new > old or (self._flush_up == 2 and new != old):
                self.flush_wgrad()
        self._wgrad_jobs.append((x, dy, dw, db))
        if post is not None:
            self._wgrad_posts.append(post)
        self._wgrad_zero += zero
        if len(self._wgrad_jobs) >= self.wgrad_batch_max:
            self.flush_wgrad()

    def wgrad_padded(self, x, dy, dw, db, post, zero):
        if self.batch_wgrad and ops.wgrad_batch_eligible(x, dy, 3, PTI_CONV_S1, PTI_PRO_NONE):
            self.defer_wgrad(x, dy, dw, db, post, zero)
            return
        with self.side_stream(x, dy, dw, db) as workspace:
            for t in zero:
                t.zero_()
            ops.conv_wgrad_mfma(x, dy, dw, db, accumulate=True, workspace=workspace)
            post()

    def flush_wgrad(self):
        jobs, self._wgrad_jobs = self._wgrad_jobs, []
        posts, self._wgrad_posts = self._wgrad_posts, []
        zero, self._wgrad_zero = self._wgrad_zero, ()
        if jobs:
            with self.side_stream(*(t for job in jobs for t in job)) as workspace:
                for t in zero:
                    t.zero_()
                ops.conv_wgrad_mfma_batched(jobs, workspace=workspace)
                for p in posts:
                    p()
        queue, self._ready_queue = self._ready_queue, []
        for rng in queue:
            self._emit_ready(rng)

    def join_wgrad(self):
        self.flush_wgrad()
        if self.wgrad_stream is not None and self._wgrad_pending:
            ev = torch.cuda.Event()
            ev.record(self.wgrad_stream)
            torch.cuda.current_stream().wait_event(ev)
            self._wgrad_pending = False

    def _ready(self, *prefixes):
        cb = self.grad_ready_cb
        if cb is None:
            return
        rng = self._range_cache.get(prefixes)
        if rng is None:
            lo, hi = None, None
            for name, (o, n, _) in self.net._slots.items():
                if name.startswith(prefixes):
                    lo = o if lo is None else min(lo, o)
                    hi = o + (n + 3) // 4 * 4 if hi is None else max(hi, o + (n + 3) // 4 * 4)
            rng = self._range_cache[prefixes] = (lo, hi)
        if rng[0] is None:
            return
        if self._wgrad_jobs or self._ready_queue:
            self._ready_queue.append(rng)
            if len(self._ready_queue) >= 6:
                self.flush_wgrad()
            return
        self._emit_ready(rng)

    def _emit_ready(self, rng):
        cb = self.grad_ready_cb
        if cb is None:
            return
        with self.side_stream():
            cb(*rng)

    def encode_forward(self, x, save):
        self.refresh_weights()
        x = self._check_input(x, self.net.in_channels, "encode")
        n, cin, h, w = x.shape
        down = 2 ** (len(self.net.channels) - 1)
        if h % down or w % down:
            raise ValueError(f"encode: H,W must be multiples of {down}, got {h}x{w}")
        self.begin_pass(n)
        c0 = self.net.channels[0]
        t0 = _empty((n, h, w, c0), x, self.act_dtype)
        xpad_b = None
        if self.enc_in.img_mfma:
            xpad, xpad_b = ops.pad_nchw_to_nhwc32(x, self.act_dtype, BF16 if (save and self.act_dtype != BF16) else None)
            if save and xpad_b is None:
                xpad_b = xpad
            st0 = self.new_stats(n)
            ops.conv_mfma(xpad, self.enc_in.wp_img, self.enc_in.b.data, t0, cout=c0, ksize=3, out_stats=st0, out_groups=self.G)
            a0 = _Act(t0, st0)
        else:
            ops.conv_direct(x, self.enc_in.w_tck, self.enc_in.b.data, t0, n=n, h=h, w=w, cin=cin, cout=c0, x_layout="nchw")
            a0 = _Act(t0, ops.gn_stats(t0, self.G, self.new_stats(n)))
# ... 258 lines not shown
```

### pti_ldm_vae_amd/ops.py

```python
from __future__ import annotations

import ctypes as C
import os
from collections import namedtuple

import torch

from . import _lib as L
from ._lib import (PTI_CONV_S1, PTI_CONV_S2PAD, PTI_CONV_UP2, PTI_CONV_ZINS, PTI_PRO_GN, PTI_PRO_GN_SILU,
                   PTI_PRO_NONE, ConvDesc)

BF16 = torch.bfloat16
F16 = torch.float16
F32 = torch.float32
I64 = torch.int64
I32 = torch.int32
I16 = torch.int16
STAT_SCALE = 65536.0
ACT16 = (BF16, F16)
LATENT_BWD_MAX_BLOCKS = 512
VAE_LOSS_MAX_BLOCKS = 1024
POST_QUANT_BWD_MAX_BLOCKS = 256


_raw_stream = getattr(torch._C, "_cuda_getCurrentRawStream", None)
_cur_device = getattr(torch._C, "_cuda_getDevice", None)


def _stream() -> int:
    if _raw_stream is not None and _cur_device is not None:
        return _raw_stream(_cur_device())
    return torch.cuda.current_stream().cuda_stream


def _ptr(t):
    return None if t is None else C.c_void_p(t.data_ptr())


def _chk(t, dtype, name, dims=None):
    if not t.is_cuda:
        raise ValueError(f"{name}: expected a CUDA(HIP) tensor")
    if (t.dtype not in dtype) if isinstance(dtype, tuple) else (t.dtype != dtype):
        raise TypeError(f"{name}: expected {dtype}, got {t.dtype}")
    if not t.is_contiguous():
        raise ValueError(f"{name}: must be contiguous")
    if dims is not None and t.dim() != dims:
        raise ValueError(f"{name}: expected {dims} dims, got {tuple(t.shape)}")


def _out(out, shape, dtype, device, name, chk_name=None, rank=True, msg=None):
    if out is None:
        return torch.empty(shape, dtype=dtype, device=device)
    _chk(out, dtype, chk_name or name, len(shape) if rank else None)
    if tuple(out.shape) != tuple(shape) or out.device != device:
        raise ValueError(msg or f"{name} must be {list(shape)} on {device}")
    return out


_SCRATCH = {}


def _scratch(kind, shape, floats, device, stream):
    key = (kind, device.index, stream) + tuple(shape)
    ws = _SCRATCH.get(key)
    if ws is None:
        ws = _SCRATCH[key] = torch.empty(floats, dtype=F32, device=device)
    return ws


def conv_out_hw(h, w, mode):
    if mode == PTI_CONV_S1:
        return h, w
    if mode == PTI_CONV_S2PAD:
        return (h + 1 - 3) // 2 + 1, (w + 1 - 3) // 2 + 1
    return 2 * h, 2 * w


def pack_conv_weight(ws, ksize, mode=PTI_CONV_S1, flip=False, out=None, f16=False):
    ws = list(ws) if isinstance(ws, (list, tuple)) else [ws]
    w0 = ws[0]
    cout, cin = w0.shape[0], w0.shape[1]
    for w in ws:
        _chk(w, F32, "weight")
        if w.shape[0] != cout or w.shape[1] != cin or w.numel() != cout * cin * ksize * ksize:
            raise ValueError("pack_conv_weight: inconsistent weight shapes")
    nbytes = L.lib().pti_conv_packed_bytes(cout * len(ws), cin, ksize, mode)
    if nbytes == 0:
        raise ValueError(f"pack_conv_weight: unsupported cout={cout} cin={cin} k={ksize}")
    if out is None:
        out = torch.empty(nbytes // 2, dtype=F16 if f16 else BF16, device=w0.device)
    elif out.numel() * 2 != nbytes or out.dtype != (F16 if f16 else BF16):
        raise ValueError("pack_conv_weight: bad out size")
    arr = (C.c_void_p * len(ws))(*[w.data_ptr() for w in ws])
    L.check(L.lib().pti_conv_pack_weights(arr, len(ws), _ptr(out), cout, cin, ksize, mode, int(flip), int(f16), _stream()),
            "pti_conv_pack_weights")
    return out


class DirectRepack:

    def __init__(self, entries):
        if not 1 <= len(entries) <= L.DIRECT_REPACK_MAX:
            raise ValueError(f"DirectRepack: 1..{L.DIRECT_REPACK_MAX} entries")
        self.table = L.DirectRepackTable()
        self.table.n = len(entries)
        self._keep = entries
        for i, e in enumerate(entries):
            w = e["w"]
            _chk(w, F32, "w", 4)
            cout, cin = w.shape[0], w.shape[1]
            if w.shape[2] != 3 or w.shape[3] != 3:
                raise ValueError("DirectRepack: 3x3 weights")
            for k in ("b", "w_tck", "w_tck_t", "wpad", "bpad"):
                if e.get(k) is not None:
                    _chk(e[k], F32, k)
            wpad = e.get("wpad")
            pad_cin = 0
            if wpad is not None:
                pad_cin = wpad.shape[1]
                if wpad.dim() != 4 or wpad.shape[0] < cout or pad_cin < cin or wpad.shape[2:] != w.shape[2:]:
                    raise ValueError("DirectRepack: wpad shape")
            for k, size in (("w_tck", cout * cin * 9), ("w_tck_t", cout * cin * 9), ("bpad", cout)):
                if e.get(k) is not None and e[k].numel() < size:
                    raise ValueError(f"DirectRepack: {k} too small")
            if e.get("bpad") is not None and (e.get("b") is None or e["b"].numel() != cout):
                raise ValueError("DirectRepack: bpad needs b")
            self.table.e[i] = L.DirectRepackEntry(_ptr(w), _ptr(e.get("b")), _ptr(e.get("w_tck")), _ptr(e.get("w_tck_t")),
                                                  _ptr(wpad), _ptr(e.get("bpad")), cout, cin, pad_cin, 0)

    def run(self):
        L.check(L.lib().pti_direct_repack(C.byref(self.table), _stream()), "pti_direct_repack")


def _chk_stats(t, count, name):
    _chk(t, I64, name)
    if t.numel() != count:
        raise ValueError(f"{name}: expected {count} fixed-point sums, got {t.numel()}")


def _chk_prologue(who, in_stats, gamma, beta, n, groups, cin):
    _chk_stats(in_stats, n * groups * 2, "in_stats")
    for t, nm in ((gamma, "gamma"), (beta, "beta")):
        _chk(t, F32, nm)
        if t.numel() != cin:
            raise ValueError(f"{who}: {nm} size")


KERNEL_PROFILE = None
_MODE_NAME = {PTI_CONV_S1: "s1", PTI_CONV_S2PAD: "s2", PTI_CONV_UP2: "up2", PTI_CONV_ZINS: "zins"}


def last_kernel_name() -> str:
    name = (L.lib().pti_last_kernel_name() or b"").decode()
    name = name.replace("(anonymous namespace)::", "")
    if name.startswith("void "):
        name = name[5:]
    depth = 0
    for i, ch in enumerate(name):
        if ch == "<":
            depth += 1
        elif ch == ">":
            depth -= 1
        elif ch == "(" and depth == 0:
            return name[:i].strip()
    return name.strip()


def _prof_begin(prof):
    e0, e1 = (torch.cuda.Event(enable_timing=True) for _ in range(2))
    e0.record()
    return prof, e0, e1


def _prof_end(rec, flops, nbytes, shape):
    prof, e0, e1 = rec
    e1.record()
    prof.append((last_kernel_name(), flops, nbytes, e0, e1, shape))


def stats_to_float(stats):
    return stats.double() / STAT_SCALE


def gn_stats(x, groups, stats=None):
    _chk(x, ACT16, "x", 4)
    n, h, w, c = x.shape
    if stats is None:
        stats = torch.zeros(n, groups, 2, dtype=I64, device=x.device)
    else:
        _chk_stats(stats, n * groups * 2, "stats")
    L.check(L.lib().pti_gn_stats(_ptr(x), _ptr(stats), n, h * w, c, groups, int(x.dtype == F16), _stream()),
            "pti_gn_stats")
    return stats


def conv_mfma(x, w_packed, bias, y, *, cout, ksize=3, mode=PTI_CONV_S1, prologue=PTI_PRO_NONE, in_stats=None,
              gamma=None, beta=None, groups=0, eps=1e-6, residual=None, out_stats=None, out_groups=0, act_out=None,
              pool2=False, relu=False):
    _chk(x, ACT16, "x", 4)
    _chk(y, ACT16, "y", 4)
    n, h, w, cin = x.shape
    if act_out is not None:
        _chk(act_out, BF16, "act_out", 4)
        if act_out.shape != x.shape:
            raise ValueError("conv_mfma: act_out shape")
    ho, wo = conv_out_hw(h, w, mode)
    yshape = (n, ho // 2, wo // 2, cout) if pool2 else (n, ho, wo, cout)
    if tuple(y.shape) != yshape:
        raise ValueError(f"conv_mfma: y shape {tuple(y.shape)} != {yshape}")
    if w_packed.numel() != cout * cin * ksize * ksize or w_packed.dtype not in (BF16, F16):
        raise ValueError("conv_mfma: packed weight size/dtype mismatch")
    w_f16 = w_packed.dtype == F16
    if bias is not None:
        _chk(bias, F32, "bias")
        if bias.numel() != cout:
            raise ValueError("conv_mfma: bias size")
    if prologue != PTI_PRO_NONE:
        _chk_prologue("conv_mfma", in_stats, gamma, beta, n, groups, cin)
    if residual is not None:
        _chk(residual, ACT16, "residual", 4)
        if residual.shape != y.shape or pool2:
            raise ValueError("conv_mfma: residual shape")
    if out_stats is not None:
        _chk_stats(out_stats, n * out_groups * 2, "out_stats")
    d = ConvDesc(n=n, h=h, w=w, cin=cin, ho=ho, wo=wo, cout=cout, ksize=ksize, mode=mode, prologue=prologue,
                 groups=groups, add_residual=int(residual is not None), accum_stats=int(out_stats is not None),
                 out_groups=out_groups, eps=eps, in_f16=int(x.dtype == F16),
                 res_f16=int(residual is not None and residual.dtype == F16), out_f16=int(y.dtype == F16),
                 pool2x2_out=int(pool2), w_f16=int(w_f16), relu_out=int(relu))
    prof = KERNEL_PROFILE
    rec = None if prof is None else _prof_begin(prof)
    if act_out is not None:
        L.check(L.lib().pti_conv2d_mfma_saveact(_ptr(x), _ptr(w_packed), _ptr(bias), _ptr(in_stats), _ptr(gamma),
                                                _ptr(beta), _ptr(residual), _ptr(y), _ptr(out_stats), _ptr(act_out),
                                                C.byref(d), _stream()), "pti_conv2d_mfma_saveact")
    else:
        L.check(L.lib().pti_conv2d_mfma(_ptr(x), _ptr(w_packed), _ptr(bias), _ptr(in_stats), _ptr(gamma), _ptr(beta),
                                        _ptr(residual), _ptr(y), _ptr(out_stats), C.byref(d), _stream()),
                "pti_conv2d_mfma")
    if rec is not None:
        flops = 2.0 * n * ho * wo * cout * cin * ksize * ksize * (0.25 if mode == PTI_CONV_ZINS else 1.0)
        nbytes = 2.0 * (x.numel() * (2 if act_out is not None else 1) + y.numel() * (2 if residual is not None else 1))
        kind = "conv fwd" if x.dtype == F16 or prologue != PTI_PRO_NONE else "conv dgrad"
        _prof_end(rec, flops, nbytes, (kind, cin, cout, ho, wo, ksize, _MODE_NAME[mode], n))
    return y


def _strides4(t, layout):
    s = t.stride()
    return (s[0], s[2], s[3], s[1]) if layout == "nchw" else (s[0], s[1], s[2], s[3])


def conv_direct(x, w_tck, bias, y, *, n, h, w, cin, cout, ksize=3, x_layout="nhwc", y_layout="nhwc",
                prologue=PTI_PRO_NONE, in_stats=None, gamma=None, beta=None, groups=0, eps=1e-6):
    _chk(w_tck, F32, "w_tck")
    if w_tck.numel() != ksize * ksize * cin * cout:
        raise ValueError("conv_direct: weight size")
    if x.numel() != n * h * w * cin or y.numel() != n * h * w * cout:
        raise ValueError("conv_direct: tensor sizes do not match n,h,w,cin,cout")
    if prologue != PTI_PRO_NONE:
        _chk_stats(in_stats, n * groups * 2, "in_stats")
    d = ConvDesc(n=n, h=h, w=w, cin=cin, ho=h, wo=w, cout=cout, ksize=ksize, mode=PTI_CONV_S1, prologue=prologue,
                 groups=groups, eps=eps, in_f32=int(x.dtype == F32), out_f32=int(y.dtype == F32),
                 in_f16=int(x.dtype == F16), out_f16=int(y.dtype == F16))
    d.in_stride = (C.c_int64 * 4)(*_strides4(x, x_layout))
    d.out_stride = (C.c_int64 * 4)(*_strides4(y, y_layout))
    if cout % 32 == 0 and cin <= 16:
        if y.dtype not in ACT16 or not y.is_contiguous() or y_layout != "nhwc":
            raise ValueError("conv_direct: wide output must be dense NHWC bf16/fp16")
    else:
        if x.dtype not in ACT16 or not x.is_contiguous() or x_layout != "nhwc":
            raise ValueError("conv_direct: wide input must be dense NHWC bf16/fp16")
    L.check(L.lib().pti_conv2d_direct(_ptr(x), _ptr(w_tck), _ptr(bias), _ptr(in_stats), _ptr(gamma), _ptr(beta),
                                      _ptr(y), C.byref(d), _stream()), "pti_conv2d_direct")
    return y


def wgrad_direct(wide, narrow, dw, *, n, h, w, cw, cn, ksize, sgn, narrow_layout, dw_strides, dbias_wide=None,
                 dbias_narrow=None, prologue=PTI_PRO_NONE, in_stats=None, gamma=None, beta=None, groups=0, eps=1e-6,
                 workspace=None):
    _chk(wide, ACT16, "wide", 4)
    _chk(dw, F32, "dw")
    if prologue != PTI_PRO_NONE:
        _chk_stats(in_stats, n * groups * 2, "in_stats")
    ns = (C.c_int64 * 4)(*_strides4(narrow, narrow_layout))
    ws = workspace if workspace is not None else wgrad_workspace(wide.device)
    L.check(L.lib().pti_wgrad_direct(_ptr(wide), _ptr(narrow), _ptr(dw), _ptr(dbias_wide), _ptr(dbias_narrow),
                                     _ptr(in_stats), _ptr(gamma), _ptr(beta), n, h, w, cw, cn, ksize, sgn, prologue,
                                     groups, eps, int(narrow.dtype == F32), int(wide.dtype == F16), ns, dw_strides[0],
                                     dw_strides[1],
                                     dw_strides[2], _ptr(ws), ws.numel() * 4, _stream()), "pti_wgrad_direct")
    return dw


_WS = {}


def wgrad_workspace(device, nbytes=int(os.environ.get("PTI_WGRAD_WORKSPACE_MB", "256")) << 20):
    key = (device.index if device.index is not None else torch.cuda.current_device())
    ws = _WS.get(key)
    if ws is None or ws.numel() * 4 < nbytes:
        ws = torch.empty(nbytes // 4, dtype=F32, device=device)
        _WS[key] = ws
    return ws


def conv_wgrad_mfma(x, dy, dw, dbias, *, ksize=3, mode=PTI_CONV_S1, prologue=PTI_PRO_NONE, in_stats=None, gamma=None,
                    beta=None, groups=0, eps=1e-6, accumulate=False, workspace=None):
    _chk(x, ACT16, "x", 4)
    _chk(dy, BF16, "dy", 4)
    _chk(dw, F32, "dw")
    n, h, w, cin = x.shape
    ho, wo = conv_out_hw(h, w, mode)
    cout = dy.shape[3]
    if tuple(dy.shape) != (n, ho, wo, cout):
        raise ValueError(f"conv_wgrad_mfma: dy shape {tuple(dy.shape)} != {(n, ho, wo, cout)}")
    if dw.numel() != cout * cin * ksize * ksize:
        raise ValueError("conv_wgrad_mfma: dw size")
    if dbias is not None:
        _chk(dbias, F32, "dbias")
        if dbias.numel() != cout:
            raise ValueError("conv_wgrad_mfma: dbias size")
    if prologue != PTI_PRO_NONE:
        _chk_prologue("conv_wgrad_mfma", in_stats, gamma, beta, n, groups, cin)
    ws = workspace if workspace is not None else wgrad_workspace(x.device)
    d = ConvDesc(n=n, h=h, w=w, cin=cin, ho=ho, wo=wo, cout=cout, ksize=ksize, mode=mode, prologue=prologue,
                 groups=groups, eps=eps, in_f16=int(x.dtype == F16))
    prof = KERNEL_PROFILE
    if prof is None:
        L.check(L.lib().pti_conv_wgrad_mfma(_ptr(x), _ptr(dy), _ptr(in_stats), _ptr(gamma), _ptr(beta), _ptr(dw),
                                            _ptr(dbias), _ptr(ws), ws.numel() * 4, int(accumulate), C.byref(d),
                                            _stream()), "pti_conv_wgrad_mfma")
        return dw
    splits = C.c_int(0)
    rec = _prof_begin(prof)
    L.check(L.lib().pti_conv_wgrad_mfma_partials(_ptr(x), _ptr(dy), _ptr(in_stats), _ptr(gamma), _ptr(beta), _ptr(ws),
                                                 ws.numel() * 4, C.byref(d), C.byref(splits), _stream()),
            "pti_conv_wgrad_mfma_partials")
    _prof_end(rec, 2.0 * n * ho * wo * cout * cin * ksize * ksize, 2.0 * (x.numel() + dy.numel()),
              ("conv wgrad", cin, cout, ho, wo, ksize, _MODE_NAME[mode], n))
    L.check(L.lib().pti_conv_wgrad_reduce(_ptr(ws), splits.value, _ptr(dw), _ptr(dbias), int(accumulate), C.byref(d),
                                          _stream()), "pti_conv_wgrad_reduce")
    return dw


def wgrad_batch_eligible(x, dy, ksize, mode, prologue):
    return (ksize == 3 and mode == PTI_CONV_S1 and prologue == PTI_PRO_NONE and x.dtype == BF16 and dy.dtype == BF16
            and x.shape[3] % 32 == 0 and dy.shape[3] % 32 == 0 and x.numel() * 2 < (1 << 31) and dy.numel() * 2 < (1 << 31))


def conv_wgrad_mfma_batched(jobs, workspace=None, accumulate=True):
    if not 1 <= len(jobs) <= L.WGRAD_BATCH_MAX:
        raise ValueError(f"conv_wgrad_mfma_batched: 1..{L.WGRAD_BATCH_MAX} jobs, got {len(jobs)}")
    arr = (L.WgradJob * len(jobs))()
    for i, (x, dy, dw, db) in enumerate(jobs):
        _chk(x, BF16, "x", 4)
        _chk(dy, BF16, "dy", 4)
        _chk(dw, F32, "dw")
        n, h, w, cin = x.shape
        cout = dy.shape[3]
        if tuple(dy.shape) != (n, h, w, cout) or dw.numel() != cout * cin * 9 or (db is not None and db.numel() != cout):
            raise ValueError(f"conv_wgrad_mfma_batched: job {i}: shapes")
        if db is not None:
            _chk(db, F32, "dbias")
        arr[i] = L.WgradJob(x.data_ptr(), dy.data_ptr(), dw.data_ptr(), None if db is None else db.data_ptr(), n, h, w, cin,
                            cout, int(accumulate))
    ws = workspace if workspace is not None else wgrad_workspace(jobs[0][0].device)
    prof = KERNEL_PROFILE
    if prof is None:
        L.check(L.lib().pti_conv_wgrad_mfma_batched(arr, len(jobs), _ptr(ws), ws.numel() * 4, _stream()),
                "pti_conv_wgrad_mfma_batched")
        return
    groups = {}
    for i, j in enumerate(arr):
        groups.setdefault(L.lib().pti_conv_wgrad_batched_mode(j.n, j.h, j.w, j.cin, j.cout), []).append(i)
    for mode in sorted(groups, reverse=True):
        idx = groups[mode]
        sub = (L.WgradJob * len(idx))(*[arr[i] for i in idx])
        rec = _prof_begin(prof)
        L.check(L.lib().pti_conv_wgrad_mfma_batched(sub, len(idx), _ptr(ws), ws.numel() * 4, _stream()),
                "pti_conv_wgrad_mfma_batched")
        _prof_end(rec, sum(2.0 * arr[i].n * arr[i].h * arr[i].w * arr[i].cout * arr[i].cin * 9 for i in idx),
                  sum(2.0 * (jobs[i][0].numel() + jobs[i][1].numel()) for i in idx),
                  ("conv wgrad (batched)", 0, 0, 0, 0, 3, "s1", len(idx)))


def gn_bwd(x, da, dx, stats, gamma, beta, sums, dgamma, dbeta, *, groups, eps=1e-6, silu=True, dres=None):
    _chk(x, ACT16, "x", 4)
    _chk(da, BF16, "da", 4)
    _chk(dx, BF16, "dx", 4)
    n, h, w, c = x.shape
    if da.shape != x.shape or dx.shape != x.shape or (dres is not None and dres.shape != x.shape):
        raise ValueError("gn_bwd: shape mismatch")
    _chk_stats(stats, n * groups * 2, "stats")
    if sums.numel() != n * c * 2:
        raise ValueError("gn_bwd: scratch sizes")
    blocks = L.lib().pti_gn_bwd_blocks(n, h * w, c)
# ... 154 lines not shown
    L.check(L.lib().pti_latent_head_bwd(_ptr(h), _ptr(eps), _ptr(wm), _ptr(bm), _ptr(wl), _ptr(bl), _ptr(wp), _ptr(bp),
                                        _ptr(dzq), _ptr(dmu), _ptr(dsigma), _ptr(dh), _ptr(gwm), _ptr(gbm), _ptr(gwl),
                                        _ptr(gbl), _ptr(gwp), _ptr(gbp), _ptr(ws), b, hw, l, _stream()),
            "pti_latent_head_bwd")


def vae_loss(recon, images, mu, third, out2, d_recon, d_mu, d_third, *, l2=False, third_mode=0, kl_weight=1e-3):
    for t, nm in ((recon, "recon"), (images, "images"), (mu, "mu"), (third, "third"), (out2, "out2")):
        _chk(t, F32, nm)
    if recon.shape != images.shape or mu.shape != third.shape or out2.numel() < 2:
        raise ValueError("vae_loss: shapes")
    ws = torch.empty(2 * VAE_LOSS_MAX_BLOCKS, dtype=torch.float32, device=recon.device)
    L.check(L.lib().pti_vae_loss(_ptr(recon), _ptr(images), recon.numel(), _ptr(mu), _ptr(third), mu.numel(),
                                 recon.shape[0], _ptr(out2), _ptr(d_recon), _ptr(d_mu), _ptr(d_third), _ptr(ws), int(l2),
                                 third_mode, kl_weight, _stream()), "pti_vae_loss")


def ar_vae_loss(mu, attrs, channels, deltas, per_attr, counts, *, gamma=0.0, d_mu=None, pair_mask=None):
    _chk(mu, F32, "mu", 4)
    _chk(attrs, F32, "attrs", 2)
    _chk(deltas, F32, "deltas")
    _chk(per_attr, F32, "per_attr")
    b, l, h, w = mu.shape
    na = attrs.shape[0]
    if attrs.shape[1] != b or channels.numel() != na or deltas.numel() != na or per_attr.numel() != na or counts.numel() != na:
        raise ValueError("ar_vae_loss: attrs must be [na, b]; channels / deltas / per_attr / counts [na]")
    if channels.dtype != torch.int32 or counts.dtype != torch.int32 or not (channels.is_cuda and counts.is_cuda):
        raise TypeError("ar_vae_loss: channels / counts must be int32 device tensors")
    if d_mu is not None:
        _chk(d_mu, F32, "d_mu", 4)
        if d_mu.shape != mu.shape:
            raise ValueError("ar_vae_loss: d_mu shape")
    if pair_mask is not None:
        if pair_mask.dtype != torch.uint8 or tuple(pair_mask.shape) != (na, b, b) or not pair_mask.is_cuda or not pair_mask.is_contiguous():
            raise ValueError("ar_vae_loss: pair_mask must be a contiguous uint8 device tensor [na, b, b]")
    L.check(L.lib().pti_ar_vae_loss(_ptr(mu), b, l, h * w, _ptr(attrs), _ptr(channels), _ptr(deltas), na, _ptr(pair_mask),
                                    float(gamma), _ptr(per_attr), _ptr(counts), _ptr(d_mu), _stream()), "pti_ar_vae_loss")


def adam_step(p, g, m, v, *, lr, beta1=0.9, beta2=0.999, eps=1e-8, step=1, grad_scale=1.0):
    for t, nm in ((p, "p"), (g, "g"), (m, "m"), (v, "v")):
        _chk(t, F32, nm)
        if t.numel() != p.numel():
            raise ValueError("adam_step: size mismatch")
    L.check(L.lib().pti_adam_step(_ptr(p), _ptr(g), _ptr(m), _ptr(v), p.numel(), lr, beta1, beta2, eps, step,
                                  grad_scale, _stream()), "pti_adam_step")


GRAD_GUARD_COLUMNS = L.GRAD_GUARD_COLUMNS
GRAD_GUARD_HOST_COLUMNS = L.GRAD_GUARD_HOST_COLUMNS
GRAD_GUARD_PARTIALS_CAP = L.GRAD_GUARD_PARTIALS_CAP


def grad_guard_ctl(device):
    return torch.zeros(len(GRAD_GUARD_COLUMNS), dtype=torch.float64, device=device)


def _chk_ctl(who, ctl, device):
    if not isinstance(ctl, torch.Tensor):
        raise ValueError(f"{who}: ctl: expected a CUDA(HIP) tensor")
    _chk(ctl, torch.float64, "ctl", 1)
    if ctl.numel() != len(GRAD_GUARD_COLUMNS) or ctl.device != device:
        raise ValueError(f"{who}: ctl must be fp64 [{len(GRAD_GUARD_COLUMNS)}] on {device}")


def grad_guard(g, *, ctl, grad_scale=1.0, max_norm=None, skip_nonfinite=False, betas=(0.9, 0.999), ema_decay=None):
    _chk(g, F32, "g", 1)
    _chk_ctl("grad_guard", ctl, g.device)
    n = g.numel()
    nparts = L.lib().pti_grad_guard_partials(n)
    stream = _stream()
    ws, _ = _scratch_bytes("grad_guard", "grad_guard", (n,), 16 * nparts, (n,), g.device, stream)
    prof = KERNEL_PROFILE
    rec = None if prof is None else _prof_begin(prof)
    L.check(L.lib().pti_grad_guard(_ptr(g), n, float(grad_scale), 0.0 if max_norm is None else float(max_norm),
                                   int(bool(skip_nonfinite)), betas[0], betas[1], 0.0 if ema_decay is None else float(ema_decay),
                                   _ptr(ws), _ptr(ctl), stream), "pti_grad_guard")
    if rec is not None:
        _prof_end(rec, 2.0 * n, 4.0 * n + 32.0 * nparts, ("grad_guard", n))
    return ws


def adam_step_guarded(p, g, m, v, *, ctl, lr, betas=(0.9, 0.999), eps=1e-8, ema=None):
    for t, nm in ((p, "p"), (g, "g"), (m, "m"), (v, "v")) + (((ema, "ema"),) if ema is not None else ()):
        _chk(t, F32, nm)
        if t.numel() != p.numel():
            raise ValueError("adam_step_guarded: size mismatch")
    _chk_ctl("adam_step_guarded", ctl, p.device)
    n = p.numel()
    prof = KERNEL_PROFILE
    rec = None if prof is None else _prof_begin(prof)
    L.check(L.lib().pti_adam_step_guarded(_ptr(p), _ptr(g), _ptr(m), _ptr(v), _ptr(ema), n, lr, betas[0], betas[1], eps,
                                          _ptr(ctl), _stream()), "pti_adam_step_guarded")
    if rec is not None:
        _prof_end(rec, 12.0 * n, (28.0 if ema is None else 36.0) * n, ("adam_step_guarded", n, ema is not None))


def cast_nchw_f32_to_nhwc_bf16(x, y):
    n, c = x.shape[0], x.shape[1]
    _chk(x, F32, "x")
    _chk(y, BF16, "y")
    L.check(L.lib().pti_cast_nchw_f32_to_nhwc_bf16(_ptr(x), _ptr(y), n, c, x.numel() // (n * c), _stream()), "cast")
    return y


def cast_nhwc_bf16_to_nchw_f32(x, y):
    n, c = y.shape[0], y.shape[1]
    _chk(x, BF16, "x")
    _chk(y, F32, "y")
    L.check(L.lib().pti_cast_nhwc_bf16_to_nchw_f32(_ptr(x), _ptr(y), n, c, y.numel() // (n * c), _stream()), "cast")
    return y


def attention_fwd(qkv, o, lse2):
    _chk(qkv, BF16, "qkv", 3)
    _chk(o, BF16, "o", 3)
    _chk(lse2, F32, "lse2")
    b, l, c3 = qkv.shape
    c = c3 // 3
    if tuple(o.shape) != (b, l, c) or lse2.numel() != b * l or c3 != 3 * c:
        raise ValueError("attention_fwd: shapes")
    L.check(L.lib().pti_attention_fwd(_ptr(qkv), _ptr(o), _ptr(lse2), b, l, c, _stream()), "pti_attention_fwd")
    return o


def attention_bwd(qkv, o, dout, lse2, delta, dqkv):
    _chk(qkv, BF16, "qkv", 3)
    _chk(o, BF16, "o", 3)
    _chk(dout, BF16, "dout", 3)
    _chk(dqkv, BF16, "dqkv", 3)
    b, l, c3 = qkv.shape
    c = c3 // 3
    if o.shape != dout.shape or tuple(o.shape) != (b, l, c) or dqkv.shape != qkv.shape:
        raise ValueError("attention_bwd: shapes")
    if lse2.numel() != b * l or delta.numel() != b * l:
        raise ValueError("attention_bwd: lse/delta sizes")
    L.check(L.lib().pti_attention_bwd(_ptr(qkv), _ptr(o), _ptr(dout), _ptr(lse2), _ptr(delta), _ptr(dqkv), b, l, c,
                                      _stream()), "pti_attention_bwd")
    return dqkv


class BatchedPacker:

    def __init__(self, entries, device):
        lib = L.lib()
        esz = lib.pti_conv_pack_entry_bytes()
        host = bytearray(esz * len(entries))
        hbuf = (C.c_char * len(host)).from_buffer(host)
        first, total, self.outputs = [], 0, []
        for i, (w, ksize, mode, flip, *rest) in enumerate(entries):
            f16 = bool(rest[0]) if rest else False
            _chk(w, F32, "weight")
            cout, cin = w.shape[0], w.shape[1]
            out = torch.empty(w.numel(), dtype=F16 if f16 else BF16, device=device)
            nb = C.c_int64(0)
            L.check(lib.pti_conv_pack_table_fill(C.byref(hbuf, i * esz), _ptr(w), _ptr(out), cout, cin, ksize, mode,
                                                 int(flip), int(f16), C.byref(nb)), "pti_conv_pack_table_fill")
            first.append(total)
            total += nb.value
            self.outputs.append(out)
        self.n, self.total_blocks = len(entries), total
        self.table = torch.frombuffer(host, dtype=torch.uint8).clone().to(device)
        self.first = torch.tensor(first, dtype=torch.int32, device=device)
        self._keep = [e[0] for e in entries]

    def run(self):
        L.check(L.lib().pti_conv_pack_weights_batched(_ptr(self.table), _ptr(self.first), self.n, self.total_blocks,
                                                      _stream()), "pti_conv_pack_weights_batched")


def preprocess_batch(src, offsets, hw, out, stats=None):
    _chk(src, F32, "src")
    _chk(out, F32, "out", 4)
    b, _, hp, wp = out.shape
    if offsets.dtype != torch.int64 or hw.dtype != torch.int32 or offsets.numel() != b or hw.numel() != 2 * b:
        raise ValueError("preprocess_batch: offsets must be int64 [B], hw int32 [B,2]")
    if not (offsets.is_cuda and hw.is_cuda and offsets.is_contiguous() and hw.is_contiguous()):
        raise ValueError("preprocess_batch: descriptor tables must be contiguous device tensors")
    if stats is None:
        stats = torch.empty(3 * b, dtype=torch.float64, device=out.device)
    L.check(L.lib().pti_preprocess_batch(_ptr(src), _ptr(offsets), _ptr(hw), b, hp, wp, _ptr(out), _ptr(stats), _stream()),
            "pti_preprocess_batch")
    return out


def _tensor(t, dtype, name, dims=None):
    if not isinstance(t, torch.Tensor):
        raise ValueError(f"{name}: expected a CUDA(HIP) tensor")
    _chk(t, dtype, name, dims)


def _dense_rows(t, name, dtype=F32, *, square=False, copy=False):
    if not isinstance(t, torch.Tensor) or not t.is_cuda:
        raise ValueError(f"{name}: expected a CUDA(HIP) tensor")
    if copy and not t.is_floating_point():
        raise TypeError(f"{name}: expected a floating-point matrix, got {t.dtype}")
    if not copy and t.dtype != dtype:
        raise TypeError(f"{name}: expected {dtype}, got {t.dtype}")
    want = (f"{name}: expected {'a square [n, n]' if square else 'an [m, n]'} matrix {'that is not empty' if copy else 'with dense rows'}, "
            f"got {tuple(t.shape)}")
    if t.dim() != 2 or (square and t.shape[0] != t.shape[1]) or (copy and 0 in t.shape):
        raise ValueError(want)
    if copy and t.dtype != dtype:
        t = t.to(dtype)
    if t.stride(1) != 1 or t.stride(0) < t.shape[1]:
        if not copy:
            raise ValueError(want)
        t = t.contiguous()
    return t


def _rows_out(out, shape, dtype, device, name):
    if out is None:
        return torch.empty(shape, dtype=dtype, device=device)
    _dense_rows(out, f"{name}: out", dtype)
    if tuple(out.shape) != tuple(shape) or out.device != device:
        raise ValueError(f"{name}: out must be {list(shape)} on {device}")
    return out


def _outs(who, out, names):
    if out is None:
        return (None,) * len(names)
    if len(out) != len(names):
        raise ValueError(f"{who}: out must be ({', '.join(names)})")
    return tuple(out)


def _scratch_bytes(who, kind, shape, nbytes, what, device, stream):
    if nbytes <= 0:
        raise ValueError(f"{who}: unsupported shape {what}")
    ws = _scratch(kind, shape, (nbytes + 3) // 4, device, stream)
    return ws, ws.numel() * 4


def _offsets(who, name, seg, device, what, host=False):
    if not isinstance(seg, torch.Tensor) or (seg.device != device and (seg.is_cuda or not host)):
        raise ValueError(f"{who}: {name} must be a CUDA(HIP) tensor on {device}")
    if seg.dtype != I32:
        raise TypeError(f"{who}: {name} must be int32, got {seg.dtype}")
    if seg.dim() != 1 or seg.numel() < 2 or not seg.is_contiguous():
        raise ValueError(f"{who}: {name} must be a contiguous vector of {what} + 1 offsets")


def _latent_attrs(who, z, attrs):
    for name, t in (("z", z), ("attrs", attrs)):
        if not isinstance(t, torch.Tensor) or not t.is_cuda:
            raise ValueError(f"{who}: {name}: expected a CUDA(HIP) tensor")
        if not t.is_floating_point():
            raise TypeError(f"{who}: {name}: expected a floating-point matrix, got {t.dtype}")
        if t.dim() != 2:
            raise ValueError(f"{who}: {name}: expected a matrix, got {tuple(t.shape)}")
    n, l = z.shape
    na = attrs.shape[0]
    if attrs.shape[1] != n or attrs.device != z.device:
        raise ValueError(f"{who}: z {tuple(z.shape)} needs attrs [na, {n}] on {z.device}, got {tuple(attrs.shape)} on {attrs.device}")
    zt, attrs = _dense_rows(z.t(), f"{who}: z", copy=True), _dense_rows(attrs, f"{who}: attrs", copy=True)
    return zt, attrs, n, l, na, (zt.stride(0) if l > 1 else n), (attrs.stride(0) if na > 1 else n)
SSIM_WINDOW, SSIM_SIGMA = 11, 1.5
_ssim_taps = None


def ssim_taps() -> torch.Tensor:
    global _ssim_taps
    if _ssim_taps is None:
        coords = torch.arange(SSIM_WINDOW) - SSIM_WINDOW // 2
        g = torch.exp(-(coords ** 2) / (2 * SSIM_SIGMA * SSIM_SIGMA))
        _ssim_taps = (g / g.sum()).to(F32).contiguous()
    return _ssim_taps


def image_metrics(pred, target, *, clamp=None, data_range=1.0, k1=0.01, k2=0.03, out=None):
    if not (pred.is_cuda and target.is_cuda):
        raise ValueError("image_metrics: expected CUDA(HIP) tensors")
    if pred.dim() != 4 or pred.shape != target.shape:
        raise ValueError(f"image_metrics: expected two [n, c, h, w] tensors of one shape, got {tuple(pred.shape)} / {tuple(target.shape)}")
    if not (pred.is_floating_point() and target.is_floating_point()):
        raise TypeError("image_metrics: expected floating-point images")
    pred, target = pred.to(F32).contiguous(), target.to(F32).contiguous()
    n, c, h, w = pred.shape
    floats = L.lib().pti_image_metrics_ws_floats(n, c, h, w)
    if floats <= 0:
        raise ValueError(f"image_metrics: unsupported shape {tuple(pred.shape)}")
    out = _out(out, (n, 4), F32, pred.device, "image_metrics: out", chk_name="out")
    stream = _stream()
    ws = _scratch("metrics", (n, c, h, w), floats, pred.device, stream)
    lo, hi = (0.0, 0.0) if clamp is None else (float(clamp[0]), float(clamp[1]))
    L.check(L.lib().pti_image_metrics(_ptr(pred), _ptr(target), n, c, h, w, int(clamp is not None), lo, hi, float(data_range),
                                      float(k1), float(k2), C.c_void_p(ssim_taps().data_ptr()), _ptr(out), _ptr(ws), stream),
            "pti_image_metrics")
    return out


def latent_pairwise(a, b=None, *, mode="dist", center=None, out=None):
    if mode not in ("dist", "dot"):
        raise ValueError(f"latent_pairwise: mode must be 'dist' or 'dot', got {mode!r}")
    a = _dense_rows(a, "latent_pairwise: a", copy=True)
    b = a if b is None else _dense_rows(b, "latent_pairwise: b", copy=True)
    if b.shape[1] != a.shape[1] or b.device != a.device:
        raise ValueError(f"latent_pairwise: a {tuple(a.shape)} and b {tuple(b.shape)} must share columns and device")
    n1, d = a.shape
    n2 = b.shape[0]
    if center is not None:
        if not isinstance(center, torch.Tensor) or not center.is_cuda:
            raise ValueError("latent_pairwise: center must be a CUDA(HIP) tensor")
        if not center.is_floating_point():
            raise TypeError("latent_pairwise: center must be floating-point")
# ... 1170 lines not shown
```

Baseline: 2697 images/s.

## Route stride-2 convs through polyphase 2x2 gathers for forward and dgrad

Adds PHASE_IN and PHASE_OUT conv modes that split a 3x3 stride-2 conv, and its zero-inserted transpose, into four 2x2 polyphase sub-convolutions with pre-summed packed weights. In the forward pass the input is decimated into phases, and in dgrad each output phase gets its own grid slice. This avoids the wasted zero-tap MFMA work of the ZINS dgrad path, which does 4x useless multiplies, and uses 16-tap weights in place of 9 (more MACs forward but a regular gather). It adds extra packed weight buffers and new kernel instantiations, and it is on by default for all S2PAD convs.

```diff
diff --git a/include/pti_vae.h b/include/pti_vae.h
--- a/include/pti_vae.h
+++ b/include/pti_vae.h
@@ -20,6 +20,8 @@
 #define PTI_CONV_S2PAD 1
 #define PTI_CONV_UP2 2
 #define PTI_CONV_ZINS 3
+#define PTI_CONV_PHASE_OUT 4
+#define PTI_CONV_PHASE_IN 5
 
 #define PTI_PRO_NONE 0
 #define PTI_PRO_GN 1
diff --git a/pti_ldm_vae_amd/_lib.py b/pti_ldm_vae_amd/_lib.py
--- a/pti_ldm_vae_amd/_lib.py
+++ b/pti_ldm_vae_amd/_lib.py
@@ -19,6 +19,7 @@
 
 ABI_VERSION = 5
 PTI_CONV_S1, PTI_CONV_S2PAD, PTI_CONV_UP2, PTI_CONV_ZINS = 0, 1, 2, 3
+PTI_CONV_PHASE_OUT, PTI_CONV_PHASE_IN = 4, 5
 PTI_PRO_NONE, PTI_PRO_GN, PTI_PRO_GN_SILU = 0, 1, 2
 
 
diff --git a/pti_ldm_vae_amd/csrc/conv_mfma.hip b/pti_ldm_vae_amd/csrc/conv_mfma.hip
--- a/pti_ldm_vae_amd/csrc/conv_mfma.hip
+++ b/pti_ldm_vae_amd/csrc/conv_mfma.hip
@@ -288,9 +288,12 @@
   }
 }
 
-template <int KS, int CK, int CT, int PXF, bool SAVE, int FM, int PRO>
+template <int KS, int CK, int CT, int PXF, bool SAVE, int FM, int PRO, int PH = 0>
 __global__ __launch_bounds__(256, (PXF == 2 ? 4 : 2)) void conv_mfma2_kernel(ConvArgs a) {
   using C = Cfg2<KS, CK, CT, PXF>;
+  static_assert(PH == 0 || (KS == 3 && !SAVE && (PRO == PTI_PRO_NONE || PRO == -1) && FM != 3), "phase gathers: plain 3x3 launches");
+  constexpr int KBC = PH ? 4 * C::KPC : C::KBC;
+  constexpr int R = PH ? (PXF == 2 ? 4 : 8) : C::R;
   const int prologue = PRO >= 0 ? PRO : a.prologue;
   const bool gn_on = FM == 3 ? true : (FM == 0 ? a.gn_mode != 0 : false);
   const bool in_f16 = FM == 0 ? (bool)a.in_f16 : (FM == 1);
@@ -308,8 +311,12 @@
   const int tile_y = t % a.tiles_y;
   const int n = t / a.tiles_y;
   const int oy0 = tile_y * C::TH2, ox0 = tile_x * C::TW2;
-  const int ct = blockIdx.y;
-  const int nchunks = a.Cin / CK;
+  const int wct = blockIdx.y;
+  const int tpp = a.Cout / CT;
+  const int oph = PH == 1 ? wct / tpp : 0;
+  const int ct = PH == 1 ? wct - oph * tpp : wct;
+  const int cchunks = a.Cin / CK;
+  const int nchunks = PH == 2 ? 4 * cchunks : cchunks;
   const int wm = wave / C::WN, wn = wave % C::WN;
 
   const int pad_lo = (a.mode == PTI_CONV_ZINS) ? 2 : (KS - 1) / 2;
@@ -372,13 +379,15 @@
 
   for (int chunk = 0; chunk < nchunks; ++chunk) {
     const unsigned char* wlane =
-        a.w + ((size_t)(ct * nchunks + chunk) * C::KBC * C::NT + wn) * 1024 + lane * 16;
-    bf16x8 wa[C::R], wb[C::R];
-    auto wload = [&](bf16x8 (&dst)[C::R], int g) {
-#pragma unroll
-      for (int u = 0; u < C::R; ++u) {
-        int kb = g * C::R + u;
-        kb = kb < C::KBC ? kb : C::KBC - 1;
+        a.w + ((size_t)(wct * nchunks + chunk) * KBC * C::NT + wn) * 1024 + lane * 16;
+    const int iph = PH == 2 ? chunk / cchunks : 0;
+    const int cch = PH == 2 ? chunk - iph * cchunks : chunk;
+    bf16x8 wa[R], wb[R];
+    auto wload = [&](bf16x8 (&dst)[R], int g) {
+#pragma unroll
+      for (int u = 0; u < R; ++u) {
+        int kb = g * R + u;
+        kb = kb < KBC ? kb : KBC - 1;
         dst[u] = *(const bf16x8*)(wlane + (size_t)kb * C::NT * 1024);
       }
     };
@@ -393,7 +402,7 @@
           const_cast<bf16*>(a.x), 0, (unsigned)a.N * (unsigned)a.H * (unsigned)a.W * (unsigned)a.Cin * 2u, 0x00020000);
       const __amdgpu_buffer_rsrc_t x2rs = __builtin_amdgcn_make_buffer_rsrc(
           const_cast<bf16*>(PRO == PRO_GNB ? a.x2 : a.x), 0, (unsigned)a.N * (unsigned)a.H * (unsigned)a.W * (unsigned)a.Cin * 2u, 0x00020000);
-      const unsigned base = ((unsigned)n * a.H * a.W * a.Cin + chunk * CK + lc * 8) * 2u;
+      const unsigned base = ((unsigned)n * a.H * a.W * a.Cin + cch * CK + lc * 8) * 2u;
       const unsigned rowb = (unsigned)a.W * a.Cin * 2u, pixb = (unsigned)a.Cin * 2u;
 #pragma unroll
       for (int it = 0; it < C::HITERS; ++it) {
@@ -402,7 +411,11 @@
         const int vy = vy0 + hy, vx = vx0 + hx;
         bool v = (p < C::NP) && (unsigned)vy < (unsigned)VH && (unsigned)vx < (unsigned)VW;
         int iy = vy, ix = vx;
-        if (twox) {
+        if constexpr (PH == 2) {
+          iy = 2 * vy + (iph >> 1);
+          ix = 2 * vx + (iph & 1);
+          v = (p < C::NP) && vy >= 0 && vx >= 0 && iy < VH && ix < VW;
+        } else if (twox) {
           if (a.mode == PTI_CONV_ZINS) v = v && !((vy | vx) & 1);
           iy = vy >> 1;
           ix = vx >> 1;
@@ -434,7 +447,7 @@
       gnb_d = -rstd * c1 - gnb_b * mean;
     } else if (prologue != PTI_PRO_NONE) {
       float mu_[8], rs_[8];
-      gn_params<8>(sfl, a.gamma, a.beta, chunk * CK + lc * 8, cpg, a.inv_cnt, a.eps, sc, sh, mu_, rs_);
+      gn_params<8>(sfl, a.gamma, a.beta, cch * CK + lc * 8, cpg, a.inv_cnt, a.eps, sc, sh, mu_, rs_);
     }
     if (chunk > 0) __syncthreads();
 #pragma unroll
@@ -512,9 +525,19 @@
     if constexpr (WLATE) wload(wa, 0);
     const int txl = lane & 15;
     auto baddr = [&](int kb) -> const unsigned char* {
-      kb = kb < C::KBC ? kb : C::KBC - 1;
+      kb = kb < KBC ? kb : KBC - 1;
       const int tap = kb / C::KPC, kc = kb - tap * C::KPC;
-      const int kh = (KS == 3) ? tap / 3 : 0, kw = tap - kh * KS;
+      int kh, kw;
+      if constexpr (PH == 1) {
+        kh = (tap >> 1) + (oph >> 1);
+        kw = (tap & 1) + (oph & 1);
+      } else if constexpr (PH == 2) {
+        kh = (tap >> 1) + 1 - (iph >> 1);
+        kw = (tap & 1) + 1 - (iph & 1);
+      } else {
+        kh = (KS == 3) ? tap / 3 : 0;
+        kw = tap - kh * KS;
+      }
       const int hx = txl + kw;
       const int tk = (hsel ^ ((hx >> C::KEY_SHIFT) & (C::NC - 1))) << 4;
       return halo + pbase[0] + (kh * C::HW + kw) * C::PIXB + ((kc * 32) ^ tk);
@@ -525,10 +548,10 @@
 #pragma unroll
       for (int i = 0; i < PXF; ++i) dst[i] = *(const bf16x8*)(bp + 2 * i * C::HW * C::PIXB);
     };
-    auto group = [&](const bf16x8 (&w)[C::R], int g) {
-      const int kb0 = g * C::R;
-#pragma unroll
-      for (int u = 0; u < C::R; ++u) {
+    auto group = [&](const bf16x8 (&w)[R], int g) {
+      const int kb0 = g * R;
+#pragma unroll
+      for (int u = 0; u < R; ++u) {
         if ((u & 1) == 0) {
           bread(b1, kb0 + u + 1);
 #pragma unroll
@@ -539,12 +562,13 @@
           for (int i = 0; i < PXF; ++i) acc[i] = mfma32<OPH>(w[u], b1[i], acc[i]);
         }
       }
-      if (C::R & 1) {
+      if (R & 1) {
 #pragma unroll
         for (int i = 0; i < PXF; ++i) b0[i] = b1[i];
       }
     };
-    constexpr int NG = C::KBC / C::R;
+    constexpr int NG = KBC / R;
+    static_assert(KBC % R == 0 && (NG == 1 || NG % 2 == 0), "the group loop below runs pairs of groups");
     bread(b0, 0);
     if constexpr (NG == 1) {
       group(wa, 0);
@@ -689,7 +713,8 @@
   }
   __syncthreads();
   const __amdgpu_buffer_rsrc_t yrs = __builtin_amdgcn_make_buffer_rsrc(
-      a.y, 0, ((unsigned)a.N * (unsigned)a.Ho * (unsigned)a.Wo * (unsigned)a.Cout * 2u) >> (a.pool2 ? 2 : 0), 0x00020000);
+      a.y, 0, PH == 1 ? (unsigned)a.N * (unsigned)a.Ho * (unsigned)a.Wo * (unsigned)a.Cout * 8u
+                      : ((unsigned)a.N * (unsigned)a.Ho * (unsigned)a.Wo * (unsigned)a.Cout * 2u) >> (a.pool2 ? 2 : 0), 0x00020000);
   if ((FM == 0 || FM == 2) && a.pool2) {
     constexpr int PITERS = (C::EITERS + 3) / 4;
 #pragma unroll
@@ -720,9 +745,12 @@
   for (int it = 0; it < C::EITERS; ++it) {
     const int p = epp0 + it * EPSTEP;
     const int oy = oy0 + (p >> 4), ox = ox0 + (p & 15);
-    if (oy < a.Ho && ox < a.Wo)
+    if (oy < a.Ho && ox < a.Wo) {
+      const unsigned opix = PH == 1 ? (unsigned)((n * 2 * a.Ho + 2 * oy + (oph >> 1)) * (2 * a.Wo) + 2 * ox + (oph & 1))
+                                    : (unsigned)((n * a.Ho + oy) * a.Wo + ox);
       __builtin_amdgcn_raw_buffer_store_b128(__builtin_bit_cast(bu32x4, *(const u32x4*)(etile + p * C::EPITCH + epc * 16)), yrs,
-                                             ((unsigned)((n * a.Ho + oy) * a.Wo + ox) * a.Cout + ct * CT + epc * 8) * 2u, 0, 2);
+                                             (opix * a.Cout + ct * CT + epc * 8) * 2u, 0, 2);
+    }
   }
   if (gn_on) {
     if (tid < 2 * CT) {
@@ -755,6 +783,25 @@
   const bool fwd_plain = fm == 1 && a.prologue == PTI_PRO_NONE && !a.gn_mode && !a.pool2;
   const bool dgrad = fm == 2 && a.prologue == PTI_PRO_NONE && !a.gn_mode && !a.out_stats;
   const bool dgrad_gn = fm == 3 && a.prologue == PTI_PRO_NONE && a.gn_mode && !a.out_stats && !a.pool2;
+  if (a.mode == PTI_CONV_PHASE_OUT || a.mode == PTI_CONV_PHASE_IN) {
+    if constexpr (KS == 3) {
+      if (a.mode == PTI_CONV_PHASE_OUT) {
+        grid.y *= 4;
+        if (fwd_plain) PTI_LAUNCH((conv_mfma2_kernel<KS, CK, CT, PXF, false, 1, PTI_PRO_NONE, 1>), grid, dim3(256), 0, st, a);
+        else if (a.w_f16) return 2;
+        else if (dgrad) PTI_LAUNCH((conv_mfma2_kernel<KS, CK, CT, PXF, false, 2, PTI_PRO_NONE, 1>), grid, dim3(256), 0, st, a);
+        else PTI_LAUNCH((conv_mfma2_kernel<KS, CK, CT, PXF, false, 0, -1, 1>), grid, dim3(256), 0, st, a);
+      } else {
+        if (fwd_plain) PTI_LAUNCH((conv_mfma2_kernel<KS, CK, CT, PXF, false, 1, PTI_PRO_NONE, 2>), grid, dim3(256), 0, st, a);
+        else if (a.w_f16) return 2;
+        else if (dgrad) PTI_LAUNCH((conv_mfma2_kernel<KS, CK, CT, PXF, false, 2, PTI_PRO_NONE, 2>), grid, dim3(256), 0, st, a);
+        else PTI_LAUNCH((conv_mfma2_kernel<KS, CK, CT, PXF, false, 0, -1, 2>), grid, dim3(256), 0, st, a);
+      }
+      return 0;
+    } else {
+      return 1;
+    }
+  }
   if (a.x2) {
     if constexpr (KS == 3 && PXF == 4 && CT == 128) {
       if (!(fm == 3 && a.gn_mode && a.act_out && !a.out_stats && !a.pool2 && a.mode == PTI_CONV_S1 && !a.relu_out)) return 4;
@@ -808,10 +855,55 @@
   int cout_o, cin_o;
   int ks, ck, cout_tile, flip;
   int f16;
+  int phase;
   long long total;
 };
 
+__device__ __forceinline__ void phase_taps(int phase, int p, int tr, int& lo, int& hi) {
+  lo = hi = phase == 1 ? 2 - p - 2 * tr : 2 * tr - p;
+  if (lo < 0) { lo = 0; hi = -1; }
+}
+
+__device__ __forceinline__ void pack_eight_phase(const PackArgs& p, int e8) {
+  const int NT = p.cout_tile / 32, KPC = p.ck / 16, KBC = 4 * KPC;
+  const int nch = p.cin_l / p.ck * (p.phase == 2 ? 4 : 1);
+  int r = e8;
+  const int lane = r % 64; r /= 64;
+  const int nt = r % NT; r /= NT;
+  const int kb = r % KBC; r /= KBC;
+  int chunk = r % nch;
+  int ct = r / nch;
+  int ph;
+  if (p.phase == 1) {
+    const int tpp = p.cout_l / p.cout_tile;
+    ph = ct / tpp;
+    ct -= ph * tpp;
+  } else {
+    const int cch = p.cin_l / p.ck;
+    ph = chunk / cch;
+    chunk -= ph * cch;
+  }
+  const int co = ct * p.cout_tile + nt * 32 + (lane & 31);
+  const int tap = kb / KPC, kc = kb % KPC;
+  const int ci0 = chunk * p.ck + kc * 16 + 8 * (lane >> 5);
+  int h0, h1, w0, w1;
+  phase_taps(p.phase, ph >> 1, tap >> 1, h0, h1);
+  phase_taps(p.phase, ph & 1, tap & 1, w0, w1);
+  const float* src = p.flip ? p.src[0] + ((size_t)ci0 * p.cin_o + co) * 9 : p.src[0] + ((size_t)co * p.cin_o + ci0) * 9;
+  const size_t stride = p.flip ? (size_t)p.cin_o * 9 : 9;
+  float f[8];
+#pragma unroll
+  for (int j = 0; j < 8; ++j) {
+    float s = 0.f;
+    for (int kh = h0; kh <= h1; ++kh)
+      for (int kw = w0; kw <= w1; ++kw) s += src[j * stride + kh * 3 + kw];
+    f[j] = s;
+  }
+  *(u32x4*)(p.dst + (size_t)e8 * 8) = p.f16 ? pack8f(f, true) : pack8(f);
+}
+
 __device__ __forceinline__ void pack_eight(const PackArgs& p, int e8) {
+  if (p.phase) return pack_eight_phase(p, e8);
   const int NT = p.cout_tile / 32, KPC = p.ck / 16, KBC = p.ks * p.ks * KPC, nch = p.cin_l / p.ck;
   int r = e8;
   const int lane = r % 64; r /= 64;
@@ -887,9 +979,18 @@
 }
 
 extern "C" int64_t pti_conv_packed_bytes(int cout, int cin, int ksize, int mode) {
-  (void)mode;
   if (cout <= 0 || cin <= 0 || cout % 32 || cin % 32 || (ksize != 1 && ksize != 3)) return 0;
+  if (mode == PTI_CONV_PHASE_OUT || mode == PTI_CONV_PHASE_IN) return ksize == 3 ? (int64_t)2 * cout * cin * 16 : 0;
   return (int64_t)2 * cout * cin * ksize * ksize;
+}
+
+static int pack_phase(PackArgs& p, int mode) {
+  p.phase = mode == PTI_CONV_PHASE_OUT ? 1 : (mode == PTI_CONV_PHASE_IN ? 2 : 0);
+  if (!p.phase) return 0;
+  if (p.ks != 3 || p.nsrc != 1) return -1;
+  if ((p.phase == 1) != (p.flip != 0)) return -1;
+  p.total = (long long)p.cout_l * p.cin_l * 16;
+  return 0;
 }
 
 extern "C" int pti_conv_pack_weights(const float* const* w, int nsrc, void* packed, int cout, int cin,
@@ -912,6 +1013,7 @@
   p.cout_tile = pick_cout_tile(p.cout_l);
   p.ck = (mode == PTI_CONV_S2PAD) ? pick_ck(p.cin_l, true) : pick_ck2(p.cin_l, p.cout_tile);
   p.total = (long long)p.cout_l * p.cin_l * ksize * ksize;
+  if (pack_phase(p, mode)) PTI_FAIL(PTI_EUNSUPPORTED, "pack_weights: the phase gathers pack one 3x3 stride-2 weight (PHASE_IN plain, PHASE_OUT transposed)");
   const int blocks = (int)((p.total + 2047) / 2048);
   PTI_LAUNCH(pack_weights_kernel, dim3(blocks), dim3(256), 0, (hipStream_t)s, p);
   PTI_CHECK_LAUNCH("pack_weights");
@@ -931,7 +1033,7 @@
   p.cout_tile = pick_cout_tile(p.cout_l);
   p.ck = (mode == PTI_CONV_S2PAD) ? pick_ck(p.cin_l, true) : pick_ck2(p.cin_l, p.cout_tile);
   p.total = (long long)p.cout_l * p.cin_l * ksize * ksize;
-  return 0;
+  return pack_phase(p, mode);
 }
 
 extern "C" int pti_conv_pack_entry_bytes(void) { return (int)sizeof(PackArgs); }
@@ -976,8 +1078,16 @@
   switch (d->mode) {
     case PTI_CONV_S1: eho = d->h; ewo = d->w; break;
     case PTI_CONV_S2PAD: eho = (d->h + 1 - 3) / 2 + 1; ewo = (d->w + 1 - 3) / 2 + 1; break;
-    case PTI_CONV_UP2: case PTI_CONV_ZINS: eho = 2 * d->h; ewo = 2 * d->w; break;
+    case PTI_CONV_UP2: case PTI_CONV_ZINS: case PTI_CONV_PHASE_OUT: eho = 2 * d->h; ewo = 2 * d->w; break;
+    case PTI_CONV_PHASE_IN: eho = d->h / 2; ewo = d->w / 2; break;
     default: PTI_FAIL(PTI_EUNSUPPORTED, "conv2d_mfma: mode %d", d->mode);
+  }
+  const bool phase = d->mode == PTI_CONV_PHASE_OUT || d->mode == PTI_CONV_PHASE_IN;
+  if (phase) {
+    if (d->ksize != 3 || d->prologue != PTI_PRO_NONE || d->add_residual || d->pool2x2_out || d->relu_out || gf || act_out)
+      PTI_FAIL(PTI_EUNSUPPORTED, "conv2d_mfma: the phase gathers are plain 3x3 launches (bias and fused statistics only)");
+    if (d->mode == PTI_CONV_PHASE_IN && ((d->h & 1) || (d->w & 1)))
+      PTI_FAIL(PTI_EUNSUPPORTED, "conv2d_mfma: PTI_CONV_PHASE_IN needs even input dims, got %dx%d", d->h, d->w);
   }
   if (d->ho != eho || d->wo != ewo)
     PTI_FAIL(PTI_EINVAL, "conv2d_mfma: output %dx%d does not match mode %d on %dx%d (want %dx%d)", d->ho, d->wo,
@@ -1039,6 +1149,7 @@
     PTI_FAIL(PTI_EUNSUPPORTED, "conv2d_mfma: input tensor of %lld bytes (the halo loads use 32-bit offsets: < 2 GiB)",
              (long long)d->n * d->h * d->w * d->cin * 2);
   a.tiles_x = cdiv(d->wo, TW); a.tiles_y = cdiv(d->ho, TH);
+  if (d->mode == PTI_CONV_PHASE_OUT) { a.Ho = d->h; a.Wo = d->w; }
   const int cout_tile = pick_cout_tile(d->cout);
   int rc, ck;
   if (d->mode == PTI_CONV_S2PAD) {
@@ -1046,7 +1157,7 @@
     rc = launch_ck<3, 2>(a, ck, cout_tile, (hipStream_t)s);
   } else {
     ck = pick_ck2(d->cin, cout_tile);
-    rc = (d->ksize == 3 && d->cin == 128 && d->cout == 128 && !a.x2) ? launch_conv_ws128(a, (hipStream_t)s) : 1;
+    rc = (d->ksize == 3 && d->cin == 128 && d->cout == 128 && !a.x2 && !phase) ? launch_conv_ws128(a, (hipStream_t)s) : 1;
     if (rc == 1)
       rc = d->ksize == 1 ? launch2<1>(a, ck, cout_tile, (hipStream_t)s) : launch2<3>(a, ck, cout_tile, (hipStream_t)s);
   }
diff --git a/pti_ldm_vae_amd/engine.py b/pti_ldm_vae_amd/engine.py
--- a/pti_ldm_vae_amd/engine.py
+++ b/pti_ldm_vae_amd/engine.py
@@ -9,8 +9,8 @@
 
 from . import ops
 from .models import autoencoderkl as M
-from .ops import (BF16, F32, PTI_CONV_S1, PTI_CONV_S2PAD, PTI_CONV_UP2, PTI_CONV_ZINS, PTI_PRO_GN, PTI_PRO_GN_SILU,
-                  PTI_PRO_NONE)
+from .ops import (BF16, F32, PTI_CONV_PHASE_IN, PTI_CONV_PHASE_OUT, PTI_CONV_S1, PTI_CONV_S2PAD, PTI_CONV_UP2,
+                  PTI_CONV_ZINS, PTI_PRO_GN, PTI_PRO_GN_SILU, PTI_PRO_NONE)
 
 
 class _Act:
@@ -66,6 +66,10 @@
             w = net._param_by_name[wname]
             self.cout, self.cin = w.shape[0], w.shape[1]
         self.wp = self.wpt = None
+        self.phases, self.wp_ph, self.wpt_ph = False, None, None
+
+    def _phase_route(self, h, w):
+        return self.phases and h % 2 == 0 and w % 2 == 0
 
     def _w(self):
         if self.fused:
@@ -94,7 +98,10 @@
         y = _empty((n, ho, wo, self.cout), x.t, out_dtype or eng.act_dtype)
         st = eng.new_stats(n) if want_stats else None
         g, b = (norm.weight.data, norm.bias.data) if norm is not None else (None, None)
-        ops.conv_mfma(x.t, self.wp, self.bias(), y, cout=self.cout, ksize=self.ksize, mode=self.mode, prologue=pro,
+        mode, wp = self.mode, self.wp
+        if self._phase_route(h, w) and pro == PTI_PRO_NONE and residual is None and act_out is None:
+            mode, wp = PTI_CONV_PHASE_IN, self.wp_ph
+        ops.conv_mfma(x.t, wp, self.bias(), y, cout=self.cout, ksize=self.ksize, mode=mode, prologue=pro,
                       in_stats=x.stats if pro else None, gamma=g, beta=b, groups=eng.G, eps=eng.eps,
                       residual=residual, out_stats=st, out_groups=eng.G, act_out=act_out)
         return _Act(y, st)
@@ -103,7 +110,10 @@
         n, ho, wo, _ = dy.shape
         if self.mode == PTI_CONV_S2PAD:
             out = _empty((n, 2 * ho, 2 * wo, self.cin), dy)
-            ops.conv_mfma(dy, self.wpt, None, out, cout=self.cin, ksize=3, mode=PTI_CONV_ZINS, residual=residual)
+            if self.phases and residual is None:
+                ops.conv_mfma(dy, self.wpt_ph, None, out, cout=self.cin, ksize=3, mode=PTI_CONV_PHASE_OUT)
+            else:
+                ops.conv_mfma(dy, self.wpt, None, out, cout=self.cin, ksize=3, mode=PTI_CONV_ZINS, residual=residual)
             return out
         if self.mode == PTI_CONV_UP2:
             pooled = _empty((n, ho // 2, wo // 2, self.cin), dy)
@@ -385,8 +395,10 @@
             self.dec_layers.append(self._make_layer(db[i], f"decoder.blocks.{i}"))
         self.dec_out = _DirectConv(net, f"decoder.blocks.{last}.conv", norm_prefix=f"decoder.blocks.{last - 1}")
         self.mfma_convs = [c for l in self.enc_layers + self.dec_layers for c in l.convs]
+        phases = os.environ.get("PTI_RESAMPLE_PHASES", "1") != "0"
         for c in self.mfma_convs:
             c.f16 = c.fwd_f16 and self.act_dtype == torch.float16
+            c.phases = phases and c.mode == PTI_CONV_S2PAD
         self.direct_convs = [self.enc_in, self.enc_out, self.dec_in, self.dec_out]
         self.enc_out.pack_f16 = self.act_dtype == torch.float16
         img = os.environ.get("PTI_IMG_MFMA", "1") == "1"
@@ -435,7 +447,7 @@
                                 for t in (self.net.param_arena, self.net.grad_arena, self.workspace_side)}
 
     def _pack_buffer_ids(self):
-        ids = [t.data_ptr() for c in self.mfma_convs for t in (c.wp, c.wpt) if t is not None]
+        ids = [t.data_ptr() for c in self.mfma_convs for t in (c.wp, c.wpt, c.wp_ph, c.wpt_ph) if t is not None]
         for c in self.direct_convs:
             ids += [t.data_ptr() for t in (c.w_tck, c.w_tck_t, c.wp_mfma, c.wpad, c.wp_img, c.wpt_img, c.wpad_img) if t is not None]
         return tuple(ids)
@@ -456,6 +468,10 @@
             for c in self.mfma_convs:
                 dmode = PTI_CONV_ZINS if c.mode == PTI_CONV_S2PAD else PTI_CONV_S1
                 entries += [(c._w(), c.ksize, c.mode, False, c.f16), (c._w(), c.ksize, dmode, True, False)]
+            phased = [c for c in self.mfma_convs if c.phases]
+            nplain = len(entries)
+            for c in phased:
+                entries += [(c._w(), 3, PTI_CONV_PHASE_IN, False, c.f16), (c._w(), 3, PTI_CONV_PHASE_OUT, True, False)]
             rep, targets = [], []
             for c in self.direct_convs:
                 c.alloc()
@@ -467,6 +483,8 @@
             self._packer = ops.BatchedPacker(entries, self.dev)
             for i, c in enumerate(self.mfma_convs):
                 c.wp, c.wpt = self._packer.outputs[2 * i], self._packer.outputs[2 * i + 1]
+            for i, c in enumerate(phased):
+                c.wp_ph, c.wpt_ph = self._packer.outputs[nplain + 2 * i], self._packer.outputs[nplain + 2 * i + 1]
             for c, attr, i in targets:
                 setattr(c, attr, self._packer.outputs[i])
         self._direct_repack.run()
diff --git a/pti_ldm_vae_amd/ops.py b/pti_ldm_vae_amd/ops.py
--- a/pti_ldm_vae_amd/ops.py
+++ b/pti_ldm_vae_amd/ops.py
@@ -7,8 +7,8 @@
 import torch
 
 from . import _lib as L
-from ._lib import (PTI_CONV_S1, PTI_CONV_S2PAD, PTI_CONV_UP2, PTI_CONV_ZINS, PTI_PRO_GN, PTI_PRO_GN_SILU,
-                   PTI_PRO_NONE, ConvDesc)
+from ._lib import (PTI_CONV_PHASE_IN, PTI_CONV_PHASE_OUT, PTI_CONV_S1, PTI_CONV_S2PAD, PTI_CONV_UP2, PTI_CONV_ZINS,
+                   PTI_PRO_GN, PTI_PRO_GN_SILU, PTI_PRO_NONE, ConvDesc)
 
 BF16 = torch.bfloat16
 F16 = torch.float16
@@ -73,7 +73,15 @@
         return h, w
     if mode == PTI_CONV_S2PAD:
         return (h + 1 - 3) // 2 + 1, (w + 1 - 3) // 2 + 1
+    if mode == PTI_CONV_PHASE_IN:
+        if h % 2 or w % 2:
+            raise ValueError(f"PTI_CONV_PHASE_IN needs even input dims, got {h}x{w}")
+        return h // 2, w // 2
     return 2 * h, 2 * w
+
+
+def conv_taps(ksize, mode):
+    return 16 if mode in (PTI_CONV_PHASE_OUT, PTI_CONV_PHASE_IN) else ksize * ksize
 
 
 def pack_conv_weight(ws, ksize, mode=PTI_CONV_S1, flip=False, out=None, f16=False):
@@ -208,7 +216,7 @@
     yshape = (n, ho // 2, wo // 2, cout) if pool2 else (n, ho, wo, cout)
     if tuple(y.shape) != yshape:
         raise ValueError(f"conv_mfma: y shape {tuple(y.shape)} != {yshape}")
-    if w_packed.numel() != cout * cin * ksize * ksize or w_packed.dtype not in (BF16, F16):
+    if w_packed.numel() != cout * cin * conv_taps(ksize, mode) or w_packed.dtype not in (BF16, F16):
         raise ValueError("conv_mfma: packed weight size/dtype mismatch")
     w_f16 = w_packed.dtype == F16
     if bias is not None:
@@ -242,7 +250,11 @@
         flops = 2.0 * n * ho * wo * cout * cin * ksize * ksize * (0.25 if mode == PTI_CONV_ZINS else 1.0)
         nbytes = 2.0 * (x.numel() * (2 if act_out is not None else 1) + y.numel() * (2 if residual is not None else 1))
         kind = "conv fwd" if x.dtype == F16 or prologue != PTI_PRO_NONE else "conv dgrad"
-        _prof_end(rec, flops, nbytes, (kind, cin, cout, ho, wo, ksize, _MODE_NAME[mode], n))
+        gather = _MODE_NAME.get(mode)
+        if gather is None:
+            gather = "s2" if mode == PTI_CONV_PHASE_IN else "zins"
+            flops *= 1.0 if mode == PTI_CONV_PHASE_IN else 0.25
+        _prof_end(rec, flops, nbytes, (kind, cin, cout, ho, wo, ksize, gather, n))
     return y
 
 
@@ -703,7 +715,7 @@
             f16 = bool(rest[0]) if rest else False
             _chk(w, F32, "weight")
             cout, cin = w.shape[0], w.shape[1]
-            out = torch.empty(w.numel(), dtype=F16 if f16 else BF16, device=device)
+            out = torch.empty(cout * cin * conv_taps(ksize, mode), dtype=F16 if f16 else BF16, device=device)
             nb = C.c_int64(0)
             L.check(lib.pti_conv_pack_table_fill(C.byref(hbuf, i * esz), _ptr(w), _ptr(out), cout, cin, ksize, mode,
                                                  int(flip), int(f16), C.byref(nb)), "pti_conv_pack_table_fill")
```

Result: no change. 2723 images/s, median of 6 (+1.0%).
